# ohsnyt/bzip2-rust

Measured on NVIDIA B200. Metric: compress_MBps_level9_byte_identical, higher is better.
Workload: dtype u8

## Files before the change

bzip2_rust_b200/csrc/bwt.cu:

```cuda
#include "common.cuh"
#include "sweep.cuh"

namespace {

constexpr int FB = 20;
constexpr u64 FMASK = (1ull << FB) - 1;
static_assert(BZ2B200_MAX_BLOCK < (1u << FB) - 1, "packed list fields are 20 bits");

constexpr int RT_IPT = 8;
constexpr int RT = BZ_THREADS * RT_IPT;
__device__ __forceinline__ u32 padi(u32 i) { return i + (i >> 5); }
constexpr int RT_PAD = RT + RT / 32 + 1;

#ifndef BZ_LW
#define BZ_LW 3072
#endif
constexpr int LW = BZ_LW;
constexpr int LIPT = LW / BZ_THREADS;
#ifndef BZ_LCAP
#define BZ_LCAP 1024
#endif
constexpr int LCAP = BZ_LCAP;
constexpr int LTILE = LW - LCAP;
#ifndef BZ_SCAP
#define BZ_SCAP 128
#endif
constexpr int SCAP = BZ_SCAP;
static_assert(LW % BZ_THREADS == 0 && LW <= 4096 && LCAP <= RT && LCAP * 2 <= LW && LCAP <= (1 << 11) && SCAP < LCAP && LW / (SCAP + 1) < 256, "local refinement geometry");
constexpr int LWP = LW + LW / 32 + 1;
__device__ __forceinline__ u32 padh(u32 i) { return i + 2u * (i >> 6); }
constexpr int LWH = LW + 2 * (LW / 64) + 2;

__device__ __forceinline__ u64 rot_key8(const u8 *T, u32 n, u32 s) {
    if (s + 8 <= n) {
        const u64 *w = (const u64 *)(T + (s & ~7u));
        u64 w0 = __ldg(w);
        u32 sh = (s & 7u) * 8u;
        if (sh == 0) return w0;
        u64 w1 = __ldg(w + 1);
        return (w0 >> sh) | (w1 << (64 - sh));
    }
    u64 k = 0;
    u32 p = s;
    for (int q = 0; q < 8; q++) { k |= (u64)T[p] << (8 * q); p++; if (p >= n) p = 0; }
    return k;
}

struct Tri { int a, b; u32 c; };
__device__ __forceinline__ u64 tri_pack(u32 flag, Tri v) {
    return ((u64)flag << 62) | ((u64)(u32)(v.a + 1) << 40) | ((u64)(u32)(v.b + 1) << 20) | (u64)v.c;
}
__device__ __forceinline__ Tri tri_unpack(u64 w) {
    Tri v;
    v.a = (int)((w >> 40) & FMASK) - 1; v.b = (int)((w >> 20) & FMASK) - 1; v.c = (u32)(w & FMASK);
    return v;
}
__device__ __forceinline__ u64 ld_vol64(const u64 *p) {
    u64 v;
    asm volatile("ld.volatile.global.u64 %0, [%1];" : "=l"(v) : "l"(p));
    return v;
}
__device__ __forceinline__ void st_vol64(u64 *p, u64 v) { asm volatile("st.volatile.global.u64 [%0], %1;" ::"l"(p), "l"(v) : "memory"); }

template <bool BSUM = false>
__device__ __forceinline__ Tri tile_lookback(u64 *st, u32 t, Tri agg) {
    const int lane = threadIdx.x & 31;
    const int bid = BSUM ? 0 : -1;
    Tri ex; ex.a = -1; ex.b = bid; ex.c = 0;
    if (t == 0) { if (lane == 0) st_vol64(st, tri_pack(2, agg)); return ex; }
    if (lane == 0) st_vol64(st + t, tri_pack(1, agg));
    for (int hi = (int)t - 1;;) {
        int tt = hi - lane;
        u64 w = tt >= 0 ? ld_vol64(st + tt) : ((2ull << 62) | ((u64)(u32)(bid + 1) << 20));
        u32 f = (u32)(w >> 62);
        u32 incm = __ballot_sync(0xffffffffu, f == 2);
        u32 nrm = __ballot_sync(0xffffffffu, f == 0);
        u32 need = incm ? ((2u << (__ffs(incm) - 1)) - 1u) : 0xffffffffu;
        if (nrm & need) continue;
        Tri v = tri_unpack(w);
        if (!((need >> lane) & 1u)) { v.a = -1; v.b = bid; v.c = 0; }
#pragma unroll
        for (int o = 16; o; o >>= 1) {
            v.a = max(v.a, __shfl_xor_sync(0xffffffffu, v.a, o));
            int ob = __shfl_xor_sync(0xffffffffu, v.b, o);
            v.b = BSUM ? v.b + ob : max(v.b, ob);
            v.c += __shfl_xor_sync(0xffffffffu, v.c, o);
        }
        ex.a = max(ex.a, v.a); ex.b = BSUM ? ex.b + v.b : max(ex.b, v.b); ex.c += v.c;
        if (incm) break;
        hi -= 32;
    }
    Tri inc; inc.a = max(ex.a, agg.a); inc.b = BSUM ? ex.b + agg.b : max(ex.b, agg.b); inc.c = ex.c + agg.c;
    if (lane == 0) st_vol64(st + t, tri_pack(2, inc));
    return ex;
}

struct RefineArgs {
    const u8 *T; const u32 *len;
    const u32 *cnt;
    u32 *SA; u32 *RANK;
    const u64 *LIN; u64 *LOUT;
    u32 *cnt_out;
    u64 *LOUT2;
    u32 *cnt_out2;
    u64 *tstate;
    u32 *ticket;
    u32 stride, rtiles, tiles_x, nblk, group;
    u32 depth_after;
};

__device__ __forceinline__ bool ticket_tile(const RefineArgs &a, u32 *s_ticket, u32 &b, u32 &t) {
    if (threadIdx.x == 0) *s_ticket = atomicAdd(a.ticket, 1u);
    __syncthreads();
    u32 ticket = *s_ticket;
    u32 per_group = a.group * a.tiles_x;
    u32 g = ticket / per_group, r = ticket - g * per_group;
    t = r / a.group;
    b = g * a.group + (r - t * a.group);
    return b < a.nblk;
}

#ifndef BZ_REFINE_MINB
#define BZ_REFINE_MINB 5
#endif
__global__ void __launch_bounds__(BZ_THREADS, BZ_REFINE_MINB) k_init_ranks(RefineArgs a) {
    __shared__ u64 sk[RT + 2];
    __shared__ __align__(8) u8 fl[RT + 8];
    __shared__ u32 hd[RT_PAD];
    __shared__ u16 ls[RT];
    __shared__ int wsi[8];
    __shared__ u32 wsu[8];
    __shared__ u32 s_ticket;
    __shared__ Tri s_ex;
    __shared__ int s_big[2];
    u32 b, t;
    if (!ticket_tile(a, &s_ticket, b, t)) return;
    const u32 n = a.len[b];
    const u32 base = t * RT;
    if (base >= n) return;
    const int tid = threadIdx.x;
    const size_t ob = (size_t)b * a.stride;
    const u8 *Tb = a.T + ob;
    const u32 *sa = a.SA + ob;
    u32 s[RT_IPT];
#pragma unroll
    for (int r = 0; r < RT_IPT; r++) {
        u32 e = r * BZ_THREADS + tid, j = base + e;
        s[r] = 0;
        if (j < n) { s[r] = __ldg(sa + j); sk[e + 1] = rot_key8(Tb, n, s[r]); }
    }
    if (tid == 0 && base > 0) sk[0] = rot_key8(Tb, n, sa[base - 1]);
    if (tid == 32 && base + RT < n) sk[RT + 1] = rot_key8(Tb, n, sa[base + RT]);
    __syncthreads();
    for (u32 e = tid; e <= RT; e += BZ_THREADS) {
        u32 j = base + e;
        fl[e] = (j == 0 || j >= n || sk[e + 1] != sk[e]) ? 1 : 0;
    }
    __syncthreads();
    const u32 eb = tid * RT_IPT;
    const u64 f8 = *(const u64 *)(fl + eb);
    const u32 f9 = fl[eb + 8];
    u32 fm = 0;
#pragma unroll
    for (int r = 0; r < RT_IPT; r++) fm |= (u32)((f8 >> (8 * r)) & 1) << r;
    int last = -1;
    u32 hmask = 0, umask = 0;
#pragma unroll
    for (int r = 0; r < RT_IPT; r++) {
        u32 j = base + eb + r;
        bool h = (fm >> r) & 1;
        bool hn = (r == RT_IPT - 1) ? (f9 != 0) : ((fm >> (r + 1)) & 1);
        if (j < n) {
            if (h) { last = (int)j; hmask |= 1u << r; }
            if (!(h && hn)) umask |= 1u << r;
        }
    }
    int tl, fe;
    int head = block_excl_max(last, wsi, tl);
    int nxa = block_excl_min_rev(fm ? (int)(eb + __ffs(fm) - 1) : 0x7fffffff, wsi, fe);
    const bool cont = fl[RT] == 0;
    if (tid == 64) {
        int big = 0;
        if (fl[0] == 0) {
            if (fe == 0x7fffffff && cont) big = 1;
            else {
                long long E = (long long)base + (fe == 0x7fffffff ? (int)RT : fe);
                long long q = E - 1 - LCAP;
                if (q >= (long long)base) big = 1;
                else if (q >= 0) big = rot_key8(Tb, n, sa[q]) == sk[1];
            }
        }
        s_big[0] = big;
    }
    if (tid == 96) {
        int big = 0;
        if (cont) {
            if (tl < 0) big = 1;
            else {
                u32 P = (u32)tl + LCAP;
                if (P < base + RT) big = 1;
                else if (P < n) big = rot_key8(Tb, n, sa[P]) == sk[RT];
            }
        }
        s_big[1] = big;
    }
    __syncthreads();
    const int nx_out = f9 ? (int)(eb + 8) : (nxa != 0x7fffffff ? nxa : (cont ? 0x7fffffff : (int)RT));
    u32 bmask = 0, nloc = 0, nbig = 0;
#pragma unroll
    for (int r = 0; r < RT_IPT; r++) {
        if ((umask >> r) & 1) {
            u32 below = fm & ((2u << r) - 1u);
            int hh = below ? (int)(base + eb + 31 - __clz(below)) : head;
            u32 above = fm >> (r + 1);
            int nx = above ? (int)(eb + r + __ffs(above)) : nx_out;
            bool big;
            if (hh < 0) big = s_big[0] != 0;
            else if (nx == 0x7fffffff) big = s_big[1] != 0;
            else big = (int)base + nx - hh > LCAP;
            if (big) { bmask |= 1u << r; nbig++; } else nloc++;
        }
    }
    u32 tot;
    u32 kk = block_excl_sum(nloc | (nbig << 16), wsu, tot);
    const u32 tloc = tot & 0xffffu, tbig = tot >> 16;
    if (tid < 32) {
        Tri agg; agg.a = tl; agg.b = (int)tbig; agg.c = tloc;
        Tri ex = tile_lookback<true>(a.tstate + (size_t)b * a.rtiles, t, agg);
        if (tid == 0) {
            s_ex = ex;
            if (base + RT >= n) {
                bool done = a.depth_after >= n;
                a.cnt_out[b] = done ? 0u : ex.c + tloc;
                a.cnt_out2[b] = done ? 0u : (u32)ex.b + tbig;
            }
        }
    }
    __syncthreads();
    head = max(head, s_ex.a);
    u32 kl = kk & 0xffffu, kb = kk >> 16;
#pragma unroll
    for (int r = 0; r < RT_IPT; r++) {
        u32 e = eb + r;
        if ((hmask >> r) & 1) head = (int)(base + e);
        hd[padi(e)] = (u32)head;
        u16 v = 0xffff;
        if ((umask >> r) & 1) v = ((bmask >> r) & 1) ? (u16)(0x8000u | kb++) : (u16)(kl++);
        ls[e] = v;
    }
    __syncthreads();
    u32 *rank = a.RANK + ob;
    u64 *lout = a.LOUT + ob + s_ex.c;
    u64 *lout2 = a.LOUT2 + ob + (u32)s_ex.b;
#pragma unroll
    for (int r = 0; r < RT_IPT; r++) {
        u32 e = r * BZ_THREADS + tid, j = base + e;
        if (j < n) {
            u32 h = hd[padi(e)];
            rank[s[r]] = h;
            u32 slot = ls[e];
            if (slot != 0xffffu) {
                u64 v = ((u64)h << (2 * FB)) | s[r];
                if (slot & 0x8000u) lout2[slot & 0x7fffu] = v; else lout[slot] = v;
            }
        }
    }
}

template <bool HIST>
__global__ void __launch_bounds__(BZ_THREADS) k_list_key(const u32 *cntp, const u32 *len, const u32 *RANK, u64 *LIST,
                                                         u32 *counts, u32 stride, u32 h) {
    u32 b = blockIdx.y, cnt = cntp[b], n = len[b];
    u32 base = blockIdx.x * BZ_TILE;
    if (base >= cnt) return;
    __shared__ u32 hist[HIST ? 5 : 1][256];
    if (HIST) {
        for (int i = threadIdx.x; i < 5 * 256; i += BZ_THREADS) (&hist[0][0])[i] = 0;
        __syncthreads();
    }
    size_t ob = (size_t)b * stride;
    u64 *list = LIST + ob;
    const u32 *rank = RANK + ob;
    u32 hh = h >= n ? h % n : h;
#pragma unroll 4
    for (int r = 0; r < BZ_IPT; r++) {
        u32 k = base + r * BZ_THREADS + threadIdx.x;
        if (k < cnt) {
            u64 x = list[k];
            u32 p = (u32)(x & FMASK) + hh;
            if (p >= n) p -= n;
            x = (x & ~(FMASK << FB)) | ((u64)__ldg(rank + p) << FB);
            list[k] = x;
            if (HIST) {
#pragma unroll
                for (int q = 0; q < 5; q++) atomicAdd(&hist[q][(u32)(x >> (FB + 8 * q)) & 255u], 1u);
            }
        }
    }
    if (HIST) {
        __syncthreads();
        for (int i = threadIdx.x; i < 5 * 256; i += BZ_THREADS) {
            u32 v = (&hist[0][0])[i];
            if (v) atomicAdd(&counts[(size_t)b * 8 * 256 + i], v);
        }
    }
}

__global__ void __launch_bounds__(BZ_THREADS, BZ_REFINE_MINB > 5 ? 5 : BZ_REFINE_MINB) k_list_refine(RefineArgs a) {
    __shared__ u64 sk[RT + 2];
    __shared__ __align__(8) u8 fl[RT + 8];
    __shared__ u32 kgs[RT_PAD], kss[RT_PAD];
    __shared__ u16 ls[RT];
    __shared__ int wsi[8];
    __shared__ u32 wsu[8];
    __shared__ u32 s_ticket;
    __shared__ Tri s_ex;
    u32 b, t;
    if (!ticket_tile(a, &s_ticket, b, t)) return;
    const u32 cnt = a.cnt[b];
    const u32 base = t * RT;
    const int tid = threadIdx.x;
    if (cnt == 0 && t == 0 && tid == 0) a.cnt_out[b] = 0;
    if (base >= cnt) return;
    const size_t ob = (size_t)b * a.stride;
    const u64 *lin = a.LIN + ob;
    u64 x[RT_IPT];
#pragma unroll
    for (int r = 0; r < RT_IPT; r++) {
        u32 e = r * BZ_THREADS + tid, k = base + e;
        x[r] = 0;
        if (k < cnt) { x[r] = __ldg(lin + k); sk[e + 1] = x[r] >> FB; }
    }
    if (tid == 0 && base > 0) sk[0] = lin[base - 1] >> FB;
    if (tid == 32 && base + RT < cnt) sk[RT + 1] = lin[base + RT] >> FB;
    __syncthreads();
    for (u32 e = tid; e <= RT; e += BZ_THREADS) {
        u32 k = base + e;
        u8 f = 3;
        if (k != 0 && k < cnt) {
            u64 c = sk[e + 1], p = sk[e];
            f = (u8)((c != p ? 1 : 0) | ((c >> FB) != (p >> FB) ? 2 : 0));
        }
        fl[e] = f;
    }
    __syncthreads();
    const u32 eb = tid * RT_IPT;
    u64 f8 = *(const u64 *)(fl + eb);
    u32 f9 = fl[eb + 8];
    int la = -1, lb = -1; u32 unres = 0;
    u32 smask = 0, gmask = 0, umask = 0;
#pragma unroll
    for (int r = 0; r < RT_IPT; r++) {
        u32 k = base + eb + r;
        u32 f = (u32)(f8 >> (8 * r)) & 3u;
        u32 fn = (r == RT_IPT - 1) ? f9 : ((u32)(f8 >> (8 * r + 8)) & 3u);
        if (k < cnt) {
            if (f & 2) { la = (int)k; gmask |= 1u << r; }
            if (f & 1) { lb = (int)k; smask |= 1u << r; }
            if (!((f & 1) && (fn & 1))) { unres++; umask |= 1u << r; }
        }
    }
    int ta, tb; u32 tu;
    int kg = block_excl_max(la, wsi, ta);
    int ks = block_excl_max(lb, wsi, tb);
    u32 ko = block_excl_sum(unres, wsu, tu);
    if (tid < 32) {
        Tri agg; agg.a = ta; agg.b = tb; agg.c = tu;
        Tri ex = tile_lookback(a.tstate + (size_t)b * a.rtiles, t, agg);
        if (tid == 0) {
            s_ex = ex;
            if (base + RT >= cnt) a.cnt_out[b] = (a.depth_after >= a.len[b]) ? 0u : ex.c + tu;
        }
    }
    __syncthreads();
    kg = max(kg, s_ex.a); ks = max(ks, s_ex.b);
    const u32 kbase = s_ex.c;
#pragma unroll
    for (int r = 0; r < RT_IPT; r++) {
        u32 e = eb + r;
        if ((gmask >> r) & 1) kg = (int)(base + e);
        if ((smask >> r) & 1) ks = (int)(base + e);
        kgs[padi(e)] = (u32)kg; kss[padi(e)] = (u32)ks;
        ls[e] = ((umask >> r) & 1) ? (u16)(ko++) : (u16)0xffff;
    }
    __syncthreads();
    u32 *sa = a.SA + ob, *rank = a.RANK + ob;
    u64 *lout = a.LOUT + ob + kbase;
#pragma unroll
    for (int r = 0; r < RT_IPT; r++) {
        u32 e = r * BZ_THREADS + tid, k = base + e;
        if (k < cnt) {
            u32 g = (u32)(x[r] >> (2 * FB));
            u32 s = (u32)(x[r] & FMASK);
            u32 kgv = kgs[padi(e)], ksv = kss[padi(e)];
            u32 nh = g + (ksv - kgv);
            sa[g + (k - kgv)] = s;
            rank[s] = nh;
            u32 slot = ls[e];
            if (slot != 0xffffu) lout[slot] = ((u64)nh << (2 * FB)) | s;
        }
    }
}

constexpr size_t LOC_K_BYTES = (size_t)LW * 4;
constexpr size_t LOC_I_BYTES = ((size_t)LWH * 2 + 15) & ~(size_t)15;
constexpr size_t LOC_G_BYTES = ((size_t)LWP * 4 + 15) & ~(size_t)15;
constexpr size_t LOC_U_BYTES = ((size_t)LWH * 2 + 15) & ~(size_t)15;
constexpr size_t LOC_W_BYTES = (size_t)(LW * 4 > 8 * 256 * 4 ? LW * 4 : 8 * 256 * 4);
constexpr size_t LOC_SMEM = LOC_K_BYTES + 2 * LOC_I_BYTES + LOC_G_BYTES + LOC_U_BYTES + LOC_W_BYTES;
static_assert(LOC_K_BYTES + 2 * LOC_I_BYTES >= (size_t)LW * 8, "staging area");
#ifndef BZ_LOCAL_MINB
#define BZ_LOCAL_MINB 3
#endif
__global__ void __launch_bounds__(BZ_THREADS, BZ_LOCAL_MINB) k_refine_local(RefineArgs a, u32 *err) {
    extern __shared__ __align__(16) u8 loc_smem[];
    u32 *K = (u32 *)loc_smem;
    u16 *IDXA = (u16 *)(loc_smem + LOC_K_BYTES);
    u16 *IDXB = (u16 *)(loc_smem + LOC_K_BYTES + LOC_I_BYTES);
    u32 *GSE = (u32 *)(loc_smem + LOC_K_BYTES + 2 * LOC_I_BYTES);
    u16 *UP = (u16 *)((u8 *)GSE + LOC_G_BYTES);
    u32 *wh = (u32 *)((u8 *)UP + LOC_U_BYTES);
    __shared__ u16 MG_GS[LW / (SCAP + 1) + 4], MG_MB[LW / (SCAP + 1) + 4];
    __shared__ int wsi[8];
    __shared__ u32 wsu[8];
    __shared__ u32 s_ticket, s_prevhead;
    __shared__ Tri s_ex;
    u32 b, t;
    if (!ticket_tile(a, &s_ticket, b, t)) return;
    const u32 cnt = a.cnt[b];
    const u32 base = t * LTILE;
    const int tid = threadIdx.x, lane = tid & 31, w = tid >> 5;
    if (cnt == 0 && t == 0 && tid == 0) a.cnt_out[b] = 0;
    if (base >= cnt) return;
    const size_t ob = (size_t)b * a.stride;
    const u64 *lin = a.LIN + ob + base;
    const u32 wlen = min((u32)LW, cnt - base);
    const u32 nom = min((u32)LTILE, cnt - base);
    const int INF = 0x7fffffff;
#pragma unroll 4
    for (int r = 0; r < LIPT; r++) {
        u32 i = r * BZ_THREADS + tid;
        if (i < wlen) {
            u64 x = __ldg(lin + i);
            K[i] = (((u32)(x >> FB) & (u32)FMASK) << 12) | i;
            GSE[padi(i)] = (u32)(x >> (2 * FB));
        }
        UP[padh(i)] = 0xffffu;
    }
    if (tid == 0) s_prevhead = base > 0 ? (u32)(__ldg(lin - 1) >> (2 * FB)) : 0xffffffffu;
    __syncthreads();
    const u32 eb = tid * LIPT;
    u32 gfm = 0;
    {
        u32 prev = tid == 0 ? s_prevhead : GSE[padi(eb - 1)];
#pragma unroll 4
        for (int r = 0; r < LIPT; r++) {
            u32 i = eb + r;
            if (i < wlen) {
                u32 hc = GSE[padi(i)];
                if (hc != prev) gfm |= 1u << r;
                prev = hc;
            }
        }
    }
    int dummy;
    const int gin = block_excl_max(gfm ? (int)(eb + 31 - __clz(gfm)) : -1, wsi, dummy);
    int nout = block_excl_min_rev(gfm ? (int)(eb + __ffs(gfm) - 1) : INF, wsi, dummy);
    if (nout == INF) nout = (int)wlen;
    u32 mcount = 0, mstarts = 0, medmask = 0;
    {
        int ge = nout;
        u32 gem[LIPT];
#pragma unroll
        for (int r = LIPT - 1; r >= 0; r--) {
            gem[r] = (u32)ge;
            if ((gfm >> r) & 1u) ge = (int)(eb + r);
        }
        int gs = gin;
#pragma unroll
        for (int r = 0; r < LIPT; r++) {
            u32 i = eb + r;
            if ((gfm >> r) & 1u) gs = (int)i;
            if (i < wlen) {
                u32 v = 0xffffffffu;
                if (gs >= 0 && gs < (int)nom) {
                    v = (u32)gs | (gem[r] << 16);
                    u32 size = gem[r] - (u32)gs;
                    if (size > (u32)LCAP) atomicOr(err, 1u);
                    if (size > (u32)SCAP) { medmask |= 1u << r; mcount++; if ((u32)gs == i) mstarts++; }
                }
                GSE[padi(i)] = v;
            }
        }
    }
    u32 mtot;
    const u32 mex = block_excl_sum(mcount | (mstarts << 16), wsu, mtot);
    const u32 M = mtot & 0xffffu, nmg = mtot >> 16;
    if (medmask) {
        u32 midx = mex & 0xffffu;
        u32 mgnext = mex >> 16;
#pragma unroll 1
        for (int r = 0; r < LIPT; r++) {
            if ((medmask >> r) & 1u) {
                u32 i = eb + r;
                if ((gfm >> r) & 1u) { MG_GS[mgnext] = (u16)i; MG_MB[mgnext] = (u16)midx; mgnext++; }
                K[i] = ((mgnext - 1u) << FB) | (K[i] >> 12);
                IDXA[padh(midx)] = (u16)i;
                midx++;
            }
        }
    }
    __syncthreads();
#pragma unroll 1
    for (int r = 0; r < LIPT; r++) {
        u32 i = r * BZ_THREADS + tid;
        if (i < wlen) {
            u32 g = GSE[padi(i)];
            u32 gs = g & 0xffffu, ge = g >> 16;
            if (g != 0xffffffffu && ge - gs <= (u32)SCAP) {
                const u32 mine = K[i];
                u32 off = 0;
#pragma unroll 4
                for (u32 q = gs; q < ge; q++) off += K[q] < mine;
                UP[padh(gs + off)] = (u16)i;
            }
        }
    }
    if (M) {
        u16 *src = IDXA, *dst = IDXB;
        const int gb = nmg > 1 ? 32 - __clz((int)nmg - 1) : 0;
        const int passes = (FB + gb + 7) / 8;
        const u32 C = ((M + BZ_THREADS - 1) / BZ_THREADS) * 32;
        const u32 lt = (1u << lane) - 1u;
        u32 *whw = wh + w * 256;
        const u32 j0 = (u32)w * C + lane;
#pragma unroll 1
        for (int p = 0; p < passes; p++) {
            const int shift = 8 * p;
#pragma unroll
            for (int k = 0; k < 8; k++) wh[k * 256 + tid] = 0;
            __syncthreads();
#pragma unroll 1
            for (u32 o = 0; o < C; o += 32) {
                u32 j = j0 + o;
                bool valid = j < M;
                u32 d = valid ? (K[src[padh(j)]] >> shift) & 255u : 256u + (u32)lane;
                u32 peers = __match_any_sync(0xffffffffu, d);
                if (valid && (peers & lt) == 0) whw[d] += __popc(peers);
                __syncwarp();
            }
            __syncthreads();
            {
                u32 c[8], total = 0;
#pragma unroll
                for (int k = 0; k < 8; k++) { c[k] = wh[k * 256 + tid]; total += c[k]; }
                u32 all;
                u32 run = block_excl_sum(total, wsu, all);
#pragma unroll
                for (int k = 0; k < 8; k++) { wh[k * 256 + tid] = run; run += c[k]; }
            }
            __syncthreads();
#pragma unroll 1
            for (u32 o = 0; o < C; o += 32) {
                u32 j = j0 + o;
                bool valid = j < M;
                u32 idx = valid ? (u32)src[padh(j)] : 0u;
                u32 d = valid ? (K[idx] >> shift) & 255u : 256u + (u32)lane;
                u32 peers = __match_any_sync(0xffffffffu, d);
                u32 before = __popc(peers & lt);
                u32 old = 0;
                if (before == 0 && valid) { old = whw[d]; whw[d] = old + __popc(peers); }
                old = __shfl_sync(0xffffffffu, old, __ffs(peers) - 1);
                if (valid) dst[padh(old + before)] = (u16)idx;
                __syncwarp();
            }
            __syncthreads();
            u16 *sw = src; src = dst; dst = sw;
        }
        for (u32 j = tid; j < M; j += BZ_THREADS) {
            u32 i = src[padh(j)];
            u32 g = K[i] >> FB;
            UP[padh((u32)MG_GS[g] + (j - (u32)MG_MB[g]))] = (u16)i;
        }
    }
    __syncthreads();
    u32 tu;
    {
        u32 sfm = 0;
        u32 occ = 0;
        u32 pk = 0xffffffffu;
        if (eb > 0) {
            u32 e = UP[padh(eb - 1)];
            if (e != 0xffffu) { u32 g = GSE[padi(e)]; pk = (g >> 16) - (g & 0xffffu) > (u32)SCAP ? K[e] & (u32)FMASK : K[e] >> 12; }
        }
#pragma unroll 2
        for (int r = 0; r <= LIPT; r++) {
            u32 p = eb + r;
            u32 e = p < (u32)LW ? (u32)UP[padh(p)] : 0xffffu;
            if (e == 0xffffu) { sfm |= 1u << r; pk = 0xffffffffu; continue; }
            u32 g = GSE[padi(e)];
            u32 k2 = (g >> 16) - (g & 0xffffu) > (u32)SCAP ? K[e] & (u32)FMASK : K[e] >> 12;
            if (p == (g & 0xffffu) || k2 != pk) sfm |= 1u << r;
            pk = k2;
            occ |= 1u << r;
        }
        occ &= (1u << LIPT) - 1u;
        const u32 own = sfm & ((1u << LIPT) - 1u);
        const u32 tm = occ & ~(own & (sfm >> 1));
        const int pin = block_excl_max(own ? (int)(eb + 31 - __clz(own)) : -1, wsi, dummy);
        u32 run = block_excl_sum((u32)__popc(tm), wsu, tu);
        int ps = pin;
#pragma unroll 4
        for (int r = 0; r < LIPT; r++) {
            u32 p = eb + r;
            if ((own >> r) & 1u) ps = (int)p;
            wh[p] = run | ((p - (u32)ps) << 12) | (((tm >> r) & 1u) << 31);
            run += (tm >> r) & 1u;
        }
    }
    __syncthreads();
    if (tid < 32) {
        Tri agg; agg.a = -1; agg.b = -1; agg.c = tu;
        Tri ex = tile_lookback(a.tstate + (size_t)b * a.rtiles, t, agg);
        if (tid == 0) {
            s_ex = ex;
            if (base + LTILE >= cnt) a.cnt_out[b] = (a.depth_after >= a.len[b]) ? 0u : ex.c + tu;
        }
    }
    u64 *stg = (u64 *)loc_smem;
    u32 *sa = a.SA + ob, *rank = a.RANK + ob;
#pragma unroll 2
    for (int r = 0; r < LIPT; r++) {
        u32 p = r * BZ_THREADS + tid;
        u32 e = UP[padh(p)];
        if (e != 0xffffu) {
            u32 gs = GSE[padi(e)] & 0xffffu;
            u32 v = wh[p];
            u64 x = __ldg(lin + e);
            u32 head = (u32)(x >> (2 * FB)), s = (u32)(x & FMASK);
            u32 off = p - gs;
            u32 nh = head + off - ((v >> 12) & 0x7ffffu);
            sa[head + off] = s;
            rank[s] = nh;
            if (v >> 31) stg[v & 0xfffu] = ((u64)nh << (2 * FB)) | s;
        }
    }
    __syncthreads();
    u64 *lout = a.LOUT + ob + s_ex.c;
    for (u32 q = tid; q < tu; q += BZ_THREADS) lout[q] = stg[q];
}

__global__ void __launch_bounds__(128) k_ref_path(const u8 *T, const u32 *len, u32 stride, u32 *sais_blocks) {
    const u32 b = blockIdx.x;
    const u32 n = len[b];
    if (n <= 5000) return;
    const u8 *x = T + (size_t)b * stride;
    __shared__ u32 s_cnt;
    if (threadIdx.x == 0) s_cnt = 0;
    __syncthreads();
    const int lo = threadIdx.x * 40;
    u32 lms = 0;
    if (lo < 4999) {
        const int top = min(lo + 40, 4999);
        bool cur_s = false;
        if (top < 4999) {
            u32 c = x[top];
            int j = top + 1;
            while (j <= 4999 && x[j] == c) j++;
            cur_s = j <= 4999 && x[j] > c;
        }
        u32 prev = x[top];
        for (int k = top - 1; k >= lo; k--) {
            u32 el = x[k];
            if (el < prev) cur_s = true;
            else if (el > prev) { if (cur_s) { lms++; cur_s = false; } }
            prev = el;
        }
    }
    lms = __reduce_add_sync(0xffffffffu, lms);
    if ((threadIdx.x & 31) == 0 && lms) atomicAdd(&s_cnt, lms);
    __syncthreads();
    if (threadIdx.x == 0 && s_cnt + 1u <= 1499u) atomicAdd(sais_blocks, 1u);
}

__global__ void __launch_bounds__(256) k_used_from_hist(const u32 *counts, u32 cstride, u32 *usedbits) {
    u32 b = blockIdx.x;
    bool used = counts[(size_t)b * cstride + threadIdx.x] != 0;
    u32 m = __ballot_sync(0xffffffffu, used);
    if ((threadIdx.x & 31) == 0) usedbits[b * 8 + (threadIdx.x >> 5)] = m;
}

__global__ void __launch_bounds__(BZ_THREADS) k_bwt_out(const u8 *T, const u32 *len, const u32 *SA, const u32 *RANK,
                                                        u8 *bwt, u32 *keyout, u32 stride) {
    u32 b = blockIdx.y, n = len[b];
    size_t ob = (size_t)b * stride;
    u32 base = blockIdx.x * BZ_TILE;
    if (blockIdx.x == 0 && threadIdx.x == 0) keyout[b] = n ? RANK[ob] : 0;
#pragma unroll 4
    for (int r = 0; r < BZ_IPT; r++) {
        u32 j = base + r * BZ_THREADS + threadIdx.x;
        if (j < n) {
            u32 s = SA[ob + j];
            bwt[ob + j] = T[ob + (s == 0 ? n - 1 : s - 1)];
        }
    }
}

}

#define LAUNCH_OK()                                                  \
    do {                                                             \
        ctx->prof_end();                                             \
        cudaError_t e_ = cudaGetLastError();                         \
        if (e_ != cudaSuccess) { ctx->fail("kernel launch", e_, __FILE__, __LINE__); return BZ2B200_E_CUDA; } \
    } while (0)

int bz_bwt_batch(bz2b200_ctx *ctx, const Batch &B, u8 *d_bwt, u32 *d_key, u32 *d_usedbits) {
    if (B.nblk == 0) return BZ2B200_OK;
    if (B.max_n > BZ2B200_MAX_BLOCK || ((uintptr_t)B.T & 7u) || (B.stride & 7u)) { ctx->err = "bwt: bad batch geometry"; return BZ2B200_E_ARG; }
    cudaStream_t st = ctx->stream;
    const u64 ne_act = B.total_n;
    const size_t ne = (size_t)B.nblk * B.stride;
    const u32 min_tile = BZ_THREADS * 8;
    const u32 tiles_min = B.stride / min_tile;
    const u32 DSTRIDE = 8 * 256;
    const u32 NTICKET = 512;
    BZ_CHECK(ctx->d_SA.ensure(ne * 4));
    BZ_CHECK(ctx->d_SA2.ensure(ne * 4));
    BZ_CHECK(ctx->d_RANK.ensure(ne * 4));
    BZ_CHECK(ctx->d_KEYA.ensure(ne * 8));
    BZ_CHECK(ctx->d_KEYB.ensure(ne * 8));
    BZ_CHECK(ctx->d_thist.ensure((size_t)B.nblk * tiles_min * 256 * 4));
    BZ_CHECK(ctx->d_tagg.ensure((size_t)B.nblk * tiles_min * 8));
    BZ_CHECK(ctx->d_VALA.ensure(ne * 8));
    BZ_CHECK(ctx->d_VALB.ensure(ne * 8));
    BZ_CHECK(ctx->d_cnt.ensure((size_t)B.nblk * 4 * 4 + 16));
    BZ_CHECK(ctx->d_R.ensure(((size_t)B.nblk * DSTRIDE + NTICKET) * 4));
    BZ_CHECK(ctx->h_small.ensure((size_t)B.nblk * 8 + 64));
    u32 *d_sais = ctx->d_cnt.as<u32>() + (size_t)B.nblk * 4;
    BZ_CHECK(cudaMemsetAsync(d_sais, 0, 8, ctx->stream));
    if (!ctx->loc_attr_done) {
        BZ_CHECK(cudaFuncSetAttribute(k_refine_local, cudaFuncAttributeMaxDynamicSharedMemorySize, (int)LOC_SMEM));
        ctx->loc_attr_done = true;
    }
    u32 *SAa = ctx->d_SA.as<u32>(), *SAb = ctx->d_SA2.as<u32>(), *RANK = ctx->d_RANK.as<u32>();
    u64 *L0 = ctx->d_KEYA.as<u64>(), *L1 = ctx->d_KEYB.as<u64>();
    u64 *G0 = ctx->d_VALA.as<u64>(), *G1 = ctx->d_VALB.as<u64>();
    u32 *tstate = ctx->d_thist.as<u32>();
    u64 *rstate = ctx->d_tagg.as<u64>();
    u32 *dcounts = ctx->d_R.as<u32>();
    u32 *tickets = dcounts + (size_t)B.nblk * DSTRIDE;
    const size_t rstate_bytes = (size_t)B.nblk * tiles_min * 8;

    BZ_CHECK(cudaMemsetAsync(dcounts, 0, ((size_t)B.nblk * DSTRIDE + NTICKET) * 4, st));
    BZ_CHECK(cudaMemsetAsync(tstate, 0, (size_t)B.nblk * tiles_min * 256 * 4, st));
    u32 epoch = 0, tk = 0;
    dim3 gfull((B.max_n + BZ_TILE - 1) / BZ_TILE, B.nblk);
    static const u32 group_knob = [] { const char *e = getenv("BZ2B200_REFINE_GROUP"); u32 g = e ? (u32)atoi(e) : 4u; return g < 1 ? 1u : g; }();
    const u32 group = group_knob < (u32)B.nblk ? group_knob : (u32)B.nblk;

    ctx->prof_begin(K_BYTE_HIST, ne_act); sweep::k_byte_hist<<<gfull, BZ_THREADS, 0, st>>>(B.T, B.len, dcounts, B.stride, DSTRIDE); LAUNCH_OK();
    ctx->prof_begin(K_REF_PATH, (u64)B.nblk * 5000); k_ref_path<<<B.nblk, 128, 0, st>>>(B.T, B.len, B.stride, d_sais); LAUNCH_OK();
    if (d_usedbits) { ctx->prof_begin(K_USED, (u64)B.nblk * 1024); k_used_from_hist<<<B.nblk, 256, 0, st>>>(dcounts, DSTRIDE, d_usedbits); LAUNCH_OK(); }
    ctx->prof_begin(K_DIGIT_SCAN, (u64)B.nblk * DSTRIDE * 4); sweep::k_digit_scan<<<B.nblk * 8, 256, 0, st>>>(dcounts); LAUNCH_OK();
    u32 *bufs[2] = {SAa, SAb};
    const u32 *src = nullptr;
    for (int p = 0; p < 8; p++) {
        sweep::Args a{};
        a.T = B.T; a.len = B.len; a.cnt = B.len; a.in = src; a.out = bufs[p & 1];
        a.stride = B.stride; a.off = 7 - p; a.nblk = (u32)B.nblk;
        epoch++;
        a.dbase = dcounts; a.dbase_stride = DSTRIDE; a.tstate = tstate; a.ticket = tickets + tk++; a.epoch = epoch;
        if ((p & 1) == 0) { ctx->prof_begin(K_SWEEP_GATHER, ne_act * 9); sweep::launch<sweep::M_GATHER>(a, B.max_n, st); }
        else { ctx->prof_begin(K_SWEEP_CARRY, ne_act * 8); sweep::launch<sweep::M_CARRY>(a, B.max_n, st); }
        LAUNCH_OK();
        src = bufs[p & 1];
    }
    u32 *SA = bufs[1];

    u32 *cntL_cur = ctx->d_cnt.as<u32>(), *cntL_nxt = cntL_cur + B.nblk;
    u32 *cntB_cur = cntL_nxt + B.nblk, *cntB_nxt = cntB_cur + B.nblk;
    RefineArgs ra{};
    ra.T = B.T; ra.len = B.len; ra.SA = SA; ra.RANK = RANK; ra.stride = B.stride; ra.rtiles = tiles_min;
    ra.nblk = (u32)B.nblk; ra.group = group; ra.tstate = rstate;
    {
        BZ_CHECK(cudaMemsetAsync(rstate, 0, rstate_bytes, st));
        ra.cnt = B.len; ra.LIN = nullptr; ra.LOUT = L0; ra.cnt_out = cntL_cur; ra.LOUT2 = G0; ra.cnt_out2 = cntB_cur;
        ra.ticket = tickets + tk++;
        ra.tiles_x = (B.max_n + RT - 1) / RT; ra.depth_after = 8;
        u32 grid = ((ra.nblk + group - 1) / group) * group * ra.tiles_x;
        ctx->prof_begin(K_INIT_RANKS, ne_act * 16); k_init_ranks<<<grid, BZ_THREADS, 0, st>>>(ra); LAUNCH_OK();
    }

    u32 *h_cnt = ctx->h_small.as<u32>();
    const int passes = 5;
    u64 rounds = 0, listsum = 0, bigsum = 0;
    for (u32 h = 8;; h *= 2) {
        BZ_CHECK(cudaMemcpyAsync(h_cnt + 2 * B.nblk, d_sais, 8, cudaMemcpyDeviceToHost, st));
        BZ_CHECK(cudaMemcpyAsync(h_cnt, cntL_cur, (size_t)B.nblk * 4, cudaMemcpyDeviceToHost, st));
        BZ_CHECK(cudaMemcpyAsync(h_cnt + B.nblk, cntB_cur, (size_t)B.nblk * 4, cudaMemcpyDeviceToHost, st));
        BZ_CHECK(cudaStreamSynchronize(st));
        u32 maxl = 0, maxb = 0;
        u64 lsum = 0, bsum = 0;
        for (int b = 0; b < B.nblk; b++) {
            if (h_cnt[b] > maxl) maxl = h_cnt[b];
            if (h_cnt[B.nblk + b] > maxb) maxb = h_cnt[B.nblk + b];
            lsum += h_cnt[b]; bsum += h_cnt[B.nblk + b];
        }
        listsum += lsum + bsum; bigsum += bsum;
        if (maxl == 0 && maxb == 0) break;
        if (h >= (1u << 30)) { ctx->err = "bwt: doubling did not terminate"; return BZ2B200_E_CUDA; }
        rounds++;
        if (tk + (u32)passes + 3 > NTICKET) { BZ_CHECK(cudaMemsetAsync(tickets, 0, NTICKET * 4, st)); tk = 0; }
        if (maxl) {
            dim3 gl((maxl + BZ_TILE - 1) / BZ_TILE, B.nblk);
            ctx->prof_begin(K_LIST_KEY, lsum * 20); k_list_key<false><<<gl, BZ_THREADS, 0, st>>>(cntL_cur, B.len, RANK, L0, nullptr, B.stride, h); LAUNCH_OK();
            BZ_CHECK(cudaMemsetAsync(rstate, 0, rstate_bytes, st));
            ra.cnt = cntL_cur; ra.LIN = L0; ra.LOUT = L1; ra.cnt_out = cntL_nxt; ra.LOUT2 = nullptr; ra.cnt_out2 = nullptr;
            ra.ticket = tickets + tk++;
            ra.tiles_x = (maxl + LTILE - 1) / LTILE; ra.depth_after = 2 * h;
            u32 grid = ((ra.nblk + group - 1) / group) * group * ra.tiles_x;
            ctx->prof_begin(K_REFINE_LOCAL, lsum * 24); k_refine_local<<<grid, BZ_THREADS, LOC_SMEM, st>>>(ra, d_sais + 1); LAUNCH_OK();
            { u64 *tl = L0; L0 = L1; L1 = tl; }
        } else BZ_CHECK(cudaMemsetAsync(cntL_nxt, 0, (size_t)B.nblk * 4, st));
        if (maxb) {
            dim3 gl((maxb + BZ_TILE - 1) / BZ_TILE, B.nblk);
            BZ_CHECK(cudaMemsetAsync(dcounts, 0, (size_t)B.nblk * DSTRIDE * 4, st));
            ctx->prof_begin(K_LIST_KEY, bsum * 20); k_list_key<true><<<gl, BZ_THREADS, 0, st>>>(cntB_cur, B.len, RANK, G0, dcounts, B.stride, h); LAUNCH_OK();
            ctx->prof_begin(K_DIGIT_SCAN, (u64)B.nblk * DSTRIDE * 4); sweep::k_digit_scan<<<B.nblk * 8, 256, 0, st>>>(dcounts); LAUNCH_OK();
            if (epoch + (u32)passes > 254) {
                BZ_CHECK(cudaMemsetAsync(tstate, 0, (size_t)B.nblk * tiles_min * 256 * 4, st));
                epoch = 0;
            }
            for (int p = 0; p < passes; p++) {
                sweep::Args a{};
                a.T = B.T; a.len = B.len; a.cnt = cntB_cur; a.in = G0; a.out = G1;
                a.stride = B.stride; a.shift = FB + 8 * p; a.nblk = (u32)B.nblk;
                epoch++;
                a.dbase = dcounts + p * 256; a.dbase_stride = DSTRIDE; a.tstate = tstate; a.ticket = tickets + tk++; a.epoch = epoch;
                ctx->prof_begin(K_SWEEP_LIST, bsum * 16); sweep::launch<sweep::M_LIST>(a, maxb, st); LAUNCH_OK();
                u64 *tl = G0; G0 = G1; G1 = tl;
            }
            BZ_CHECK(cudaMemsetAsync(rstate, 0, rstate_bytes, st));
            ra.cnt = cntB_cur; ra.LIN = G0; ra.LOUT = G1; ra.cnt_out = cntB_nxt; ra.LOUT2 = nullptr; ra.cnt_out2 = nullptr;
            ra.ticket = tickets + tk++;
            ra.tiles_x = (maxb + RT - 1) / RT; ra.depth_after = 2 * h;
            u32 grid = ((ra.nblk + group - 1) / group) * group * ra.tiles_x;
            ctx->prof_begin(K_LIST_REFINE, bsum * 24); k_list_refine<<<grid, BZ_THREADS, 0, st>>>(ra); LAUNCH_OK();
            { u64 *tl = G0; G0 = G1; G1 = tl; }
        } else BZ_CHECK(cudaMemsetAsync(cntB_nxt, 0, (size_t)B.nblk * 4, st));
        { u32 *tc = cntL_cur; cntL_cur = cntL_nxt; cntL_nxt = tc; }
        { u32 *tc = cntB_cur; cntB_cur = cntB_nxt; cntB_nxt = tc; }
    }
    if (h_cnt[2 * B.nblk + 1]) { ctx->err = "bwt: a local group exceeded its capacity"; return BZ2B200_E_CUDA; }
    ctx->prof_begin(K_BWT_OUT, ne_act * 6); k_bwt_out<<<gfull, BZ_THREADS, 0, st>>>(B.T, B.len, SA, RANK, d_bwt, d_key, B.stride); LAUNCH_OK();
    ctx->bwt_stats[0] = (u64)B.nblk; ctx->bwt_stats[1] = ne_act; ctx->bwt_stats[2] = rounds; ctx->bwt_stats[3] = listsum;
    ctx->bwt_stats[4] = h_cnt[2 * B.nblk];
    ctx->bwt_stats[5] += h_cnt[2 * B.nblk];
    ctx->bwt_stats[6] += (u64)B.nblk;
    ctx->bwt_stats[7] = bigsum;
    return BZ2B200_OK;
}
```

bzip2_rust_b200/csrc/common.cuh:

```cuda
#pragma once
#include <cuda_runtime.h>
#include <stdint.h>
#include <stddef.h>
#include <mutex>
#include <string>
#include <vector>
#include <new>
#include "../../include/bz2b200.h"

typedef uint8_t u8;
typedef uint16_t u16;
typedef uint32_t u32;
typedef uint64_t u64;

#define BZ_CHECK(call)                                                                     \
    do {                                                                                   \
        cudaError_t e_ = (call);                                                           \
        if (e_ != cudaSuccess) {                                                           \
            ctx->fail(#call, e_, __FILE__, __LINE__);                                      \
            return BZ2B200_E_CUDA;                                                         \
        }                                                                                  \
    } while (0)

#define BZ_API_TRY try {
#define BZ_API_CATCH } catch (const std::bad_alloc &) { return BZ2B200_E_NOMEM; } catch (...) { return BZ2B200_E_CUDA; }

struct DevBuf {
    void *p = nullptr;
    size_t cap = 0;
    cudaError_t ensure(size_t bytes) {
        if (bytes <= cap) return cudaSuccess;
        if (p) cudaFree(p);
        p = nullptr; cap = 0;
        size_t want = bytes + bytes / 8 + 4096;
        cudaError_t e = cudaMalloc(&p, want);
        if (e == cudaSuccess) cap = want;
        return e;
    }
    void release() { if (p) cudaFree(p); p = nullptr; cap = 0; }
    template <class T> T *as() const { return (T *)p; }
};
struct PinBuf {
    void *p = nullptr;
    size_t cap = 0;
    cudaError_t ensure(size_t bytes) {
        if (bytes <= cap) return cudaSuccess;
        if (p) cudaFreeHost(p);
        p = nullptr; cap = 0;
        size_t want = bytes + bytes / 8 + 4096;
        cudaError_t e = cudaMallocHost(&p, want);
        if (e == cudaSuccess) cap = want;
        return e;
    }
    void release() { if (p) cudaFreeHost(p); p = nullptr; cap = 0; }
    template <class T> T *as() const { return (T *)p; }
};

constexpr int BZ_THREADS = 256;
constexpr int BZ_IPT = 16;
constexpr int BZ_TILE = BZ_THREADS * BZ_IPT;
constexpr int BZ_GROUP = 50;
constexpr int BZ_MAXSYM = 258;

struct Batch {
    int nblk;
    u32 stride;
    u32 tiles;
    u32 max_n;
    int nbits;
    const u8 *T;
    const u32 *len;
    u64 total_n;
};

enum KernelId { K_RADIX_HIST0, K_RADIX_SCAN, K_RADIX_SCATTER0, K_REF_PATH, K_BYTE_HIST, K_DIGIT_SCAN, K_SWEEP_GATHER, K_SWEEP_CARRY, K_SWEEP_LIST, K_INIT_RANKS, K_LIST_KEY, K_LIST_REFINE, K_REFINE_LOCAL, K_BWT_OUT, K_USED, K_MTF_SUMMARY, K_MTF_SCAN, K_MTF_EMIT, K_HUF_INIT, K_HUF_SELECT, K_HUF_LENGTHS, K_HUF_GBITS, K_HUF_LAYOUT, K_HUF_EMIT, K_RLE_SCAN, K_RLE_CHAIN, K_RLE_EMIT, K_CRC_PIECES, K_CRC_FINAL, K_CONCAT, K_FOOTER, K_DEC_MISC, K_DEC_MAGIC, K_DEC_HEADER, K_DEC_JUMPS, K_DEC_BOUNDS, K_DEC_SYMS, K_DEC_CHUNKS, K_DEC_EXPAND, K_DEC_CHUNK_SCAN, K_IBWT_CHASE, K_IBWT_RANK, K_IBWT_WRITE, K_DEC_RLE1_COUNT, K_DEC_RLE1_WRITE, K_COUNT };
static const char *const kKernelNames[] = { "k_radix_hist0", "k_radix_scan", "k_radix_scatter0", "k_ref_path", "k_byte_hist", "k_digit_scan", "k_sweep_gather", "k_sweep_carry", "k_sweep_list", "k_init_ranks", "k_list_key", "k_list_refine", "k_refine_local", "k_bwt_out", "k_used", "k_mtf_summary", "k_mtf_scan", "k_mtf_emit", "k_huf_init", "k_huf_select", "k_huf_lengths", "k_huf_gbits", "k_huf_layout", "k_huf_emit", "k_rle_scan", "k_rle_chain", "k_rle_emit", "k_crc_pieces", "k_crc_final", "k_concat", "k_footer", "k_dec_misc", "k_dec_find_magic", "k_dec_header", "k_dec_jumps", "k_dec_bounds", "k_dec_syms", "k_dec_chunks", "k_dec_expand", "k_dec_chunk_scan", "k_ibwt_chase", "k_ibwt_rank", "k_ibwt_write", "k_dec_rle1_count", "k_dec_rle1_write" };

struct KStat { double ms = 0; u64 launches = 0; u64 bytes = 0; };
struct PendingEv { int id; u64 bytes; cudaEvent_t a, b; };

struct Arrival {
    std::vector<cudaEvent_t> *ev;
    size_t chunk;
    size_t win_off;
    size_t waited;
};

struct ShardPlan {
    bool scanned = false;
    const u8 *d_win = nullptr; size_t win_lo = 0, win_len = 0, n_total = 0; int level = 0;
    bool planned = false;
    bool eof = false; u32 off_from = 0, stop_rel = 0, s0 = 0, nb = 0;
};

struct bz2b200_ctx {
    int device = 0;
    ShardPlan shard;
    cudaStream_t stream = nullptr;
    cudaStream_t s_up = nullptr, s_down = nullptr;
    std::vector<cudaEvent_t> up_ev;
    Arrival *arrival = nullptr;
    std::mutex mu;
    std::string err;
    u64 launches = 0;
    bool timing = false;
    bool dec_attr_done = false;
    bool loc_attr_done = false;
    float stage_ms[8] = {0};
    u64 bwt_stats[8] = {0};
    cudaEvent_t ev[8] = {nullptr};
    cudaEvent_t ev_total[2] = {nullptr, nullptr};
    cudaStream_t s_hi = nullptr;
    cudaEvent_t ev_dec[2] = {nullptr, nullptr};

    DevBuf d_T, d_len, d_crc;
    PinBuf h_stage, h_small, h_out;
    DevBuf d_SA, d_SA2, d_RANK, d_F, d_KEYA, d_KEYB, d_VALA, d_VALB, d_thist, d_tagg, d_cnt, d_bwt, d_key;
    DevBuf d_mtfstate, d_chunkrec, d_R, d_sym, d_m, d_freq, d_used, d_agg2;
    DevBuf d_len6, d_rfreq, d_sel, d_gbits, d_hdr, d_bitoff, d_out, d_outbits, d_hmisc;
    DevBuf d_in, d_runflag, d_misc, d_stream, d_dec1, d_dec2, d_dec3;
    DevBuf d_dwin, d_ddec[2];
    PinBuf h_dstage[2], h_dpiece[2];
    bool dstream_open = false;

    KStat kstat[K_COUNT];
    std::vector<cudaEvent_t> ev_pool;
    std::vector<PendingEv> pending;
    size_t ev_used = 0;
    int cur_id = -1;
    int prof_level = 0;
    cudaEvent_t next_event() {
        if (ev_used == ev_pool.size()) { cudaEvent_t e; cudaEventCreate(&e); ev_pool.push_back(e); }
        return ev_pool[ev_used++];
    }
    void prof_begin(int id, u64 bytes) {
        cur_id = id;
        if (prof_level < 2) return;
        PendingEv p; p.id = id; p.bytes = bytes; p.a = next_event(); p.b = next_event();
        cudaEventRecord(p.a, stream);
        pending.push_back(p);
    }
    void prof_end() {
        launches++;
        if (prof_level < 2 || pending.empty()) return;
        cudaEventRecord(pending.back().b, stream);
    }
    void prof_collect() {
        for (auto &p : pending) {
            float ms = 0;
            if (cudaEventElapsedTime(&ms, p.a, p.b) == cudaSuccess) { kstat[p.id].ms += ms; kstat[p.id].launches++; kstat[p.id].bytes += p.bytes; }
        }
        pending.clear();
        ev_used = 0;
    }

    void fail(const char *what, cudaError_t e, const char *file, int line) {
        err = std::string(what) + ": " + cudaGetErrorString(e) + " at " + file + ":" + std::to_string(line);
    }
    ~bz2b200_ctx();
};

#ifdef __CUDACC__
__device__ __forceinline__ u32 warp_incl_sum(u32 v) {
#pragma unroll
    for (int o = 1; o < 32; o <<= 1) {
        u32 t = __shfl_up_sync(0xffffffffu, v, o);
        if ((threadIdx.x & 31) >= o) v += t;
    }
    return v;
}
__device__ __forceinline__ int warp_incl_max(int v) {
#pragma unroll
    for (int o = 1; o < 32; o <<= 1) {
        int t = __shfl_up_sync(0xffffffffu, v, o);
        if ((threadIdx.x & 31) >= o) v = max(v, t);
    }
    return v;
}
__device__ __forceinline__ u32 block_excl_sum(u32 v, u32 *ws, u32 &total) {
    int lane = threadIdx.x & 31, w = threadIdx.x >> 5;
    u32 inc = warp_incl_sum(v);
    __syncthreads();
    if (lane == 31) ws[w] = inc;
    __syncthreads();
    u32 wsum = (lane < (int)(blockDim.x >> 5)) ? ws[lane] : 0;
    u32 winc = warp_incl_sum(wsum);
    u32 wbase = __shfl_sync(0xffffffffu, winc, w) - __shfl_sync(0xffffffffu, wsum, w);
    total = __shfl_sync(0xffffffffu, winc, (blockDim.x >> 5) - 1);
    return wbase + inc - v;
}
__device__ __forceinline__ int block_excl_max(int v, int *ws, int &total) {
    int lane = threadIdx.x & 31, w = threadIdx.x >> 5;
    int inc = warp_incl_max(v);
    __syncthreads();
    if (lane == 31) ws[w] = inc;
    __syncthreads();
    int wv = (lane < (int)(blockDim.x >> 5)) ? ws[lane] : -1;
    int winc = warp_incl_max(wv);
    int wprev = __shfl_up_sync(0xffffffffu, winc, 1);
    if (lane == 0) wprev = -1;
    int wbase = __shfl_sync(0xffffffffu, wprev, w);
    total = __shfl_sync(0xffffffffu, winc, (blockDim.x >> 5) - 1);
    int prev = __shfl_up_sync(0xffffffffu, inc, 1);
    if (lane == 0) prev = -1;
    return max(wbase, prev);
}
__device__ __forceinline__ int block_excl_min_rev(int v, int *ws, int &total) {
    const int INF = 0x7fffffff;
    int lane = threadIdx.x & 31, w = threadIdx.x >> 5;
    int inc = v;
#pragma unroll
    for (int o = 1; o < 32; o <<= 1) {
        int t = __shfl_down_sync(0xffffffffu, inc, o);
        if (lane + o < 32) inc = min(inc, t);
    }
    __syncthreads();
    if (lane == 0) ws[w] = inc;
    __syncthreads();
    int wv = (lane < (int)(blockDim.x >> 5)) ? ws[lane] : INF;
    int winc = wv;
#pragma unroll
    for (int o = 1; o < 32; o <<= 1) {
        int t = __shfl_down_sync(0xffffffffu, winc, o);
        if (lane + o < 32) winc = min(winc, t);
    }
    int wnext = __shfl_down_sync(0xffffffffu, winc, 1);
    if (lane == 31) wnext = INF;
    int wbase = __shfl_sync(0xffffffffu, wnext, w);
    total = __shfl_sync(0xffffffffu, winc, 0);
    int nxt = __shfl_down_sync(0xffffffffu, inc, 1);
    if (lane == 31) nxt = INF;
    return min(wbase, nxt);
}
#endif

int bz_stage_blocks(bz2b200_ctx *ctx, int nblk, const u8 *const *blk, const u32 *len, Batch &B);
int bz_make_batch_dev(bz2b200_ctx *ctx, int nblk, u32 stride, u32 max_n, const u8 *dT, const u32 *dlen, Batch &B);
int bz_bwt_batch(bz2b200_ctx *ctx, const Batch &B, u8 *d_bwt , u32 *d_key ,
                 u32 *d_usedbits = nullptr);
int bz_mtf_batch(bz2b200_ctx *ctx, const Batch &B, const u8 *d_bwt, u16 *d_sym , u32 *d_m,
                 u32 *d_freq , u8 *d_used , bool used_ready = false);
struct HufOut {
    u8 *d_out;
    u64 *d_bits;
    size_t out_stride;
    u8 *d_len6;
    u8 *d_sel;
    u32 sel_stride;
    u32 *d_ntab;
};
int bz_huf_batch(bz2b200_ctx *ctx, const Batch &B, const u16 *d_sym, const u32 *d_m, const u32 *d_freq,
                 const u8 *d_used, int emit_header, const u32 *d_crc, const u32 *d_key, HufOut &out);

int bz_rle1_window(bz2b200_ctx *ctx, const u8 *d_x, u32 W, int level, bool is_eof, u32 off_from, u32 max_blocks,
                   Batch &B, u32 *nblocks, u32 *consumed, std::vector<u32> *h_spans, bool plan_only,
                   u32 stop_at = 0xFFFFFFFFu, int skip = 0, u32 s0 = 0);
int bz_crc_dev(bz2b200_ctx *ctx, const u8 *d_x, u32 n, u32 *d_crc_out);
int bz_compress_batch(bz2b200_ctx *ctx, const Batch &B, const u32 *d_crc, HufOut &H);
int bz_contexts_on_device(int device);
std::mutex &bz_device_lock(int device);

enum { DEC_BLOCK = 0, DEC_FOOTER = 1, DEC_STREAM = 2 };
struct DecEvent {
    u64 bit;
    u32 val;
    u32 nblock;
    int kind;
};
constexpr long long DEC_ENDED = 1ll << 62;
constexpr int DEC_ABORTED = 1;
struct DecSink {
    virtual long long chain_start() { return -1; }
    virtual void chain_end(long long) {}
    virtual int counted(u64 nbytes, bool last, u8 **d_out, u8 **h_out) = 0;
    virtual int ready(const u8 *, u64) { return BZ2B200_OK; }
    virtual ~DecSink() {}
};
struct DecWindow {
    const u8 *in; size_t in_lo, n;
    const u8 *d_win; size_t lo, len;
    u64 hi_bit;
    long long expect;
    u32 combined;
    u32 max_block;
    const std::vector<u64> *cand;
};
int bz_dec_candidates(bz2b200_ctx *ctx, const u8 *d_win, size_t len, u32 cap, std::vector<u64> &cand);
void bz_add_chance_candidates(std::vector<u64> &cand);
int bz_decode_core(bz2b200_ctx *ctx, const DecWindow &w, DecSink &sink, std::vector<DecEvent> &ev);
int bz_check_block_sizes(std::string &err, int level, const std::vector<DecEvent> &ev);
```

bzip2_rust_b200/csrc/sweep.cuh:

```cuda
#pragma once
#include "common.cuh"
#include <stdlib.h>
#include <type_traits>

namespace sweep {

enum { M_GATHER = 0, M_LIST = 1, M_CARRY = 2 };

struct Args {
    const u8 *T; const u32 *len;
    const u32 *cnt;
    const void *in; void *out;
    const u32 *dbase;
    u32 dbase_stride;
    u32 *tstate;
    u32 *ticket;
    u32 stride;
    u32 rtiles;
    u32 epoch;
    u32 tiles_x;
    u32 nblk;
    u32 group;
    int off;
    int shift;
};

__device__ __forceinline__ u32 ld_vol(const u32 *p) {
    u32 v;
    asm volatile("ld.volatile.global.u32 %0, [%1];" : "=r"(v) : "l"(p));
    return v;
}
__device__ __forceinline__ void st_vol(u32 *p, u32 v) { asm volatile("st.volatile.global.u32 [%0], %1;" ::"l"(p), "r"(v) : "memory"); }

#ifndef BZ_SWEEP_TMA
#define BZ_SWEEP_TMA 0
#endif
__device__ __forceinline__ u32 smem_u32(const void *p) { return (u32)__cvta_generic_to_shared(p); }
__device__ __forceinline__ void mbar_init(u64 *bar, u32 count) {
    asm volatile("mbarrier.init.shared::cta.b64 [%0], %1;" ::"r"(smem_u32(bar)), "r"(count) : "memory");
    asm volatile("fence.mbarrier_init.release.cluster;" ::: "memory");
}
__device__ __forceinline__ void bulk_load(void *dst, const void *src, u32 bytes, u64 *bar) {
    asm volatile("mbarrier.arrive.expect_tx.shared::cta.b64 _, [%0], %1;" ::"r"(smem_u32(bar)), "r"(bytes) : "memory");
    asm volatile("cp.async.bulk.shared::cluster.global.mbarrier::complete_tx::bytes [%0], [%1], %2, [%3];"
                 ::"r"(smem_u32(dst)), "l"(src), "r"(bytes), "r"(smem_u32(bar)) : "memory");
}
__device__ __forceinline__ void mbar_wait(u64 *bar, u32 parity) {
    u32 ok;
    do {
        asm volatile("{\n .reg .pred p;\n mbarrier.try_wait.parity.shared::cta.b64 p, [%1], %2;\n selp.u32 %0, 1, 0, p;\n}"
                     : "=r"(ok) : "r"(smem_u32(bar)), "r"(parity) : "memory");
    } while (!ok);
}

template <int MODE> struct Types { typedef u32 In; typedef u32 Stage; typedef u32 Out; };
template <> struct Types<M_GATHER> { typedef u32 In; typedef u64 Stage; typedef u32 Out; };
template <> struct Types<M_LIST> { typedef u64 In; typedef u64 Stage; typedef u64 Out; };

template <int MODE, int IPT, bool FULL>
__device__ __forceinline__ void tile_body(const Args &a, u32 b, u32 t, u32 base, u32 tile_n, u32 n, u32 *wh, u32 *toff,
                                          u32 *ws, typename Types<MODE>::Stage *sbuf, u64 *bar) {
    typedef typename Types<MODE>::Stage S;
    typedef typename Types<MODE>::Out O;
    const int tid = threadIdx.x, lane = tid & 31, w = tid >> 5;
    const u32 lt = (1u << lane) - 1u;
    const u32 e0 = (u32)w * (32 * IPT) + lane;
    u32 *whw = wh + w * 256;
    typename std::conditional<MODE == M_LIST, u64, u32>::type v[IPT];
    u32 cp[MODE == M_GATHER ? (IPT + 3) / 4 : 1];
    u32 rk[IPT];

    if (MODE == M_GATHER) {
        const u32 *in = a.in ? (const u32 *)a.in + (size_t)b * a.stride + base : nullptr;
        const u8 *Tb = a.T + (size_t)b * a.stride;
        const u32 offm1 = (u32)a.off - 1u;
#pragma unroll
        for (int r = 0; r < IPT; r++) {
            u32 e = e0 + r * 32;
            v[r] = 0;
            if (FULL || e < tile_n) v[r] = in ? __ldg(in + e) : base + e;
        }
#pragma unroll
        for (int q = 0; q < (IPT + 3) / 4; q++) cp[q] = 0;
#pragma unroll
        for (int r = 0; r < IPT; r++) {
            u32 q0 = (u32)v[r] + offm1;
            if (q0 >= n) { q0 -= n; while (q0 >= n) q0 -= n; }
            u64 word = __ldg((const u64 *)(Tb + (q0 & ~7u)));
            u32 sh = (q0 & 7u) * 8u;
            u32 two = (u32)(word >> sh);
            u32 c = two & 255u, d = (two >> 8) & 255u;
            if ((q0 & 7u) == 7u || q0 + 1 >= n) d = __ldg(Tb + (q0 + 1 >= n ? 0u : q0 + 1));
            v[r] = (u32)v[r] | (d << 24);
            cp[r >> 2] |= c << (8 * (r & 3));
        }
    } else if (BZ_SWEEP_TMA && FULL) {
        mbar_wait(bar, 0);
#pragma unroll
        for (int r = 0; r < IPT; r++) v[r] = sbuf[e0 + r * 32];
    } else if (MODE == M_CARRY) {
        const u32 *in = (const u32 *)a.in + (size_t)b * a.stride + base;
#pragma unroll
        for (int r = 0; r < IPT; r++) {
            u32 e = e0 + r * 32;
            v[r] = 0;
            if (FULL || e < tile_n) v[r] = __ldg(in + e);
        }
    } else {
        const u64 *in = (const u64 *)a.in + (size_t)b * a.stride + base;
#pragma unroll
        for (int r = 0; r < IPT; r++) {
            u32 e = e0 + r * 32;
            v[r] = 0;
            if (FULL || e < tile_n) v[r] = __ldg(in + e);
        }
    }
#define SWEEP_DIGIT(x) (MODE == M_LIST ? ((u32)((u64)(x) >> a.shift) & 255u) : ((u32)(x) >> 24))
#pragma unroll
    for (int r = 0; r < IPT; r++) {
        bool valid = FULL || (e0 + r * 32 < tile_n);
        u32 d = SWEEP_DIGIT(v[r]);
        u32 peers = __match_any_sync(0xffffffffu, valid ? d : 256u);
        u32 before = __popc(peers & lt);
        u32 old = 0;
        if (before == 0 && valid) { old = whw[d]; whw[d] = old + __popc(peers); }
        old = __shfl_sync(0xffffffffu, old, __ffs(peers) - 1);
        rk[r] = old + before;
        __syncwarp();
    }
    __syncthreads();
    {
        u32 c[8], total = 0;
#pragma unroll
        for (int k = 0; k < 8; k++) { c[k] = wh[k * 256 + tid]; total += c[k]; }
        const u32 tag = a.epoch << 22;
        u32 *my = a.tstate + ((size_t)b * a.rtiles + t) * 256 + tid;
        if (t == 0) st_vol(my, (2u << 30) | tag | total);
        else st_vol(my, (1u << 30) | tag | total);
        u32 all;
        u32 ex = block_excl_sum(total, ws, all);
        u32 run = ex;
#pragma unroll
        for (int k = 0; k < 8; k++) { wh[k * 256 + tid] = run; run += c[k]; }
        u32 excl = 0;
        if (t != 0) {
            const u32 *p = my - 256;
            for (int tt = (int)t - 1; tt >= 0;) {
                u32 x = ld_vol(p);
                if (((x >> 22) & 255u) != a.epoch || (x >> 30) == 0) continue;
                excl += x & 0x3fffffu;
                if ((x >> 30) == 2u) break;
                tt--; p -= 256;
            }
            st_vol(my, (2u << 30) | tag | (excl + total));
        }
        toff[tid] = a.dbase[(size_t)b * a.dbase_stride + tid] + excl - ex;
    }
    __syncthreads();
#pragma unroll
    for (int r = 0; r < IPT; r++) {
        if (FULL || (e0 + r * 32 < tile_n)) {
            u32 d = SWEEP_DIGIT(v[r]);
            S x = (S)v[r];
            if (MODE == M_GATHER) x = (S)((u64)v[r] | ((u64)((cp[r >> 2] >> (8 * (r & 3))) & 255u) << 32));
            sbuf[whw[d] + rk[r]] = x;
        }
    }
    __syncthreads();
    O *out = (O *)a.out + (size_t)b * a.stride;
#pragma unroll
    for (int r = 0; r < IPT; r++) {
        u32 p = r * BZ_THREADS + tid;
        if (FULL || p < tile_n) {
            S x = sbuf[p];
            u32 d = SWEEP_DIGIT(x);
            O y;
            if (MODE == M_GATHER) y = (O)(((u32)x & 0xffffffu) | ((u32)((u64)x >> 32) << 24));
            else if (MODE == M_CARRY) y = (O)((u32)x & 0xffffffu);
            else y = (O)x;
            out[toff[d] + p] = y;
        }
    }
#undef SWEEP_DIGIT
}

#ifndef BZ_SWEEP_MINB_G
#define BZ_SWEEP_MINB_G 3
#endif
#ifndef BZ_SWEEP_MINB_L
#define BZ_SWEEP_MINB_L 3
#endif
constexpr int min_ctas(int MODE, int IPT) {
    return MODE == M_CARRY ? (IPT <= 8 ? 6 : 4) : (IPT <= 8 ? 4 : (MODE == M_GATHER ? BZ_SWEEP_MINB_G : BZ_SWEEP_MINB_L));
}

template <int MODE, int IPT>
__global__ void __launch_bounds__(BZ_THREADS, min_ctas(MODE, IPT)) k_sweep(Args a) {
    typedef typename Types<MODE>::Stage S;
    constexpr int TILE = BZ_THREADS * IPT;
    __shared__ u32 wh[8 * 256];
    __shared__ u32 toff[256];
    __shared__ u32 ws[8];
    __shared__ __align__(16) S sbuf[TILE];
    __shared__ __align__(8) u64 s_bar;
    __shared__ u32 s_ticket;
    const int tid = threadIdx.x;
    if (tid == 0) {
        s_ticket = atomicAdd(a.ticket, 1u);
        if (BZ_SWEEP_TMA && MODE != M_GATHER) mbar_init(&s_bar, 1);
    }
#pragma unroll
    for (int k = 0; k < 8; k++) wh[k * 256 + tid] = 0;
    __syncthreads();
    u32 ticket = s_ticket;
    u32 per_group = a.group * a.tiles_x;
    u32 g = ticket / per_group, r = ticket - g * per_group;
    u32 t = r / a.group;
    u32 b = g * a.group + (r - t * a.group);
    if (b >= a.nblk) return;
    u32 cnt = a.cnt[b];
    u32 base = t * TILE;
    if (base >= cnt) return;
    u32 n = a.len[b];
    u32 tile_n = min((u32)TILE, cnt - base);
    if (tile_n == (u32)TILE) {
        if (BZ_SWEEP_TMA && MODE != M_GATHER && tid == 0) {
            typedef typename Types<MODE>::In I;
            bulk_load(sbuf, (const I *)a.in + (size_t)b * a.stride + base, (u32)(TILE * sizeof(I)), &s_bar);
        }
        tile_body<MODE, IPT, true>(a, b, t, base, tile_n, n, wh, toff, ws, sbuf, &s_bar);
    } else tile_body<MODE, IPT, false>(a, b, t, base, tile_n, n, wh, toff, ws, sbuf, &s_bar);
}

struct Knobs { int ipt0, ipt1; u32 group, group_stream; };
static inline const Knobs &knobs() {
    static Knobs k = [] {
        Knobs q;
        const char *e;
        q.ipt0 = (e = getenv("BZ2B200_SWEEP_IPT0")) ? atoi(e) : 16;
        q.ipt1 = (e = getenv("BZ2B200_SWEEP_IPT1")) ? atoi(e) : 16;
        q.group = (e = getenv("BZ2B200_SWEEP_GROUP")) ? (u32)atoi(e) : 32u;
        q.group_stream = (e = getenv("BZ2B200_SWEEP_GROUP_STREAM")) ? (u32)atoi(e) : 128u;
        if (q.group_stream < 1) q.group_stream = 1;
        if (q.ipt0 != 8 && q.ipt0 != 16) q.ipt0 = 16;
        if (q.ipt1 != 8 && q.ipt1 != 16) q.ipt1 = 16;
        if (q.group < 1) q.group = 1;
        return q;
    }();
    return k;
}
static inline u32 tile_elems(int mode) { return (u32)(BZ_THREADS * (mode == M_LIST ? knobs().ipt1 : knobs().ipt0)); }

template <int MODE>
static inline void launch(Args a, u32 max_cnt, cudaStream_t st) {
    const Knobs &k = knobs();
    int ipt = MODE == M_LIST ? k.ipt1 : k.ipt0;
    u32 tile = (u32)(BZ_THREADS * ipt);
    a.tiles_x = (max_cnt + tile - 1) / tile;
    a.rtiles = a.stride / tile;
    a.group = MODE == M_GATHER ? k.group : k.group_stream;
    if (a.group > a.nblk) a.group = a.nblk;
    u32 grid = ((a.nblk + a.group - 1) / a.group) * a.group * a.tiles_x;
    if (grid == 0) return;
    if (ipt == 8) k_sweep<MODE, 8><<<grid, BZ_THREADS, 0, st>>>(a);
    else k_sweep<MODE, 16><<<grid, BZ_THREADS, 0, st>>>(a);
}

static __global__ void __launch_bounds__(BZ_THREADS) k_byte_hist(const u8 *T, const u32 *len, u32 *counts, u32 stride,
                                                                  u32 cstride) {
    u32 b = blockIdx.y, n = len[b];
    u32 base = blockIdx.x * BZ_TILE;
    if (base >= n) return;
    __shared__ u32 h[8][256];
    for (int i = threadIdx.x; i < 8 * 256; i += BZ_THREADS) (&h[0][0])[i] = 0;
    __syncthreads();
    const u8 *t = T + (size_t)b * stride;
    int w = threadIdx.x >> 5;
#pragma unroll 4
    for (int r = 0; r < BZ_IPT; r++) {
        u32 i = base + r * BZ_THREADS + threadIdx.x;
        if (i < n) atomicAdd(&h[w][t[i]], 1u);
    }
    __syncthreads();
    u32 s = 0;
#pragma unroll
    for (int k = 0; k < 8; k++) s += h[k][threadIdx.x];
    if (s) atomicAdd(&counts[(size_t)b * cstride + threadIdx.x], s);
}

static __global__ void __launch_bounds__(256) k_digit_scan(u32 *counts) {
    __shared__ u32 ws[8];
    u32 v = counts[(size_t)blockIdx.x * 256 + threadIdx.x], all;
    u32 ex = block_excl_sum(v, ws, all);
    counts[(size_t)blockIdx.x * 256 + threadIdx.x] = ex;
}

}
```

Baseline: 7395.

## Make init-ranks and gather sweep persistent with cp.async prefetch of next tile

Turns k_init_ranks and the gather-mode sweep into persistent kernels that loop over tickets, with the grid capped at the number of resident CTAs. While the current tile is still being processed, each CTA claims its next tile and issues cp.async loads of the text bytes that tile needs into a dynamic shared buffer. The aim is to hide the latency of the random text gathers behind the scan and scatter work of the tile in flight. In exchange it uses more shared memory (occupancy drops, init min blocks go from 5 to 4), adds double-buffered ticket slots and extra syncs, and makes the control flow more complex.

```diff
diff --git a/bzip2_rust_b200/csrc/bwt.cu b/bzip2_rust_b200/csrc/bwt.cu
--- a/bzip2_rust_b200/csrc/bwt.cu
+++ b/bzip2_rust_b200/csrc/bwt.cu
@@ -112,158 +112,198 @@
 __device__ __forceinline__ bool ticket_tile(const RefineArgs &a, u32 *s_ticket, u32 &b, u32 &t) {
     if (threadIdx.x == 0) *s_ticket = atomicAdd(a.ticket, 1u);
     __syncthreads();
-    u32 ticket = *s_ticket;
-    u32 per_group = a.group * a.tiles_x;
-    u32 g = ticket / per_group, r = ticket - g * per_group;
-    t = r / a.group;
-    b = g * a.group + (r - t * a.group);
+    sweep::ticket_to_tile(*s_ticket, a.group, a.tiles_x, b, t);
     return b < a.nblk;
 }
 
-#ifndef BZ_REFINE_MINB
-#define BZ_REFINE_MINB 5
-#endif
-__global__ void __launch_bounds__(BZ_THREADS, BZ_REFINE_MINB) k_init_ranks(RefineArgs a) {
-    __shared__ u64 sk[RT + 2];
-    __shared__ __align__(8) u8 fl[RT + 8];
-    __shared__ u32 hd[RT_PAD];
-    __shared__ u16 ls[RT];
-    __shared__ int wsi[8];
-    __shared__ u32 wsu[8];
-    __shared__ u32 s_ticket;
-    __shared__ Tri s_ex;
-    __shared__ int s_big[2];
-    u32 b, t;
-    if (!ticket_tile(a, &s_ticket, b, t)) return;
-    const u32 n = a.len[b];
-    const u32 base = t * RT;
-    if (base >= n) return;
-    const int tid = threadIdx.x;
+constexpr size_t INIT_KW_BYTES = (size_t)2 * RT * 8;
+constexpr int INIT_MINB = 4;
+static_assert(RT_PAD * 4 + RT * 2 <= (RT + 2) * 8, "hd and ls share sk's space");
+
+__device__ __forceinline__ void init_issue(const RefineArgs &a, u32 b, u32 t, u32 (&s)[RT_IPT], u64 *kw) {
+    const u32 n = a.len[b], base = t * RT;
     const size_t ob = (size_t)b * a.stride;
     const u8 *Tb = a.T + ob;
     const u32 *sa = a.SA + ob;
-    u32 s[RT_IPT];
 #pragma unroll
     for (int r = 0; r < RT_IPT; r++) {
-        u32 e = r * BZ_THREADS + tid, j = base + e;
+        u32 j = base + r * BZ_THREADS + threadIdx.x;
         s[r] = 0;
-        if (j < n) { s[r] = __ldg(sa + j); sk[e + 1] = rot_key8(Tb, n, s[r]); }
-    }
-    if (tid == 0 && base > 0) sk[0] = rot_key8(Tb, n, sa[base - 1]);
-    if (tid == 32 && base + RT < n) sk[RT + 1] = rot_key8(Tb, n, sa[base + RT]);
-    __syncthreads();
-    for (u32 e = tid; e <= RT; e += BZ_THREADS) {
-        u32 j = base + e;
-        fl[e] = (j == 0 || j >= n || sk[e + 1] != sk[e]) ? 1 : 0;
-    }
-    __syncthreads();
-    const u32 eb = tid * RT_IPT;
-    const u64 f8 = *(const u64 *)(fl + eb);
-    const u32 f9 = fl[eb + 8];
-    u32 fm = 0;
-#pragma unroll
-    for (int r = 0; r < RT_IPT; r++) fm |= (u32)((f8 >> (8 * r)) & 1) << r;
-    int last = -1;
-    u32 hmask = 0, umask = 0;
+        if (j < n) s[r] = __ldg(sa + j);
+    }
 #pragma unroll
     for (int r = 0; r < RT_IPT; r++) {
-        u32 j = base + eb + r;
-        bool h = (fm >> r) & 1;
-        bool hn = (r == RT_IPT - 1) ? (f9 != 0) : ((fm >> (r + 1)) & 1);
-        if (j < n) {
-            if (h) { last = (int)j; hmask |= 1u << r; }
-            if (!(h && hn)) umask |= 1u << r;
-        }
-    }
-    int tl, fe;
-    int head = block_excl_max(last, wsi, tl);
-    int nxa = block_excl_min_rev(fm ? (int)(eb + __ffs(fm) - 1) : 0x7fffffff, wsi, fe);
-    const bool cont = fl[RT] == 0;
-    if (tid == 64) {
-        int big = 0;
-        if (fl[0] == 0) {
-            if (fe == 0x7fffffff && cont) big = 1;
-            else {
-                long long E = (long long)base + (fe == 0x7fffffff ? (int)RT : fe);
-                long long q = E - 1 - LCAP;
-                if (q >= (long long)base) big = 1;
-                else if (q >= 0) big = rot_key8(Tb, n, sa[q]) == sk[1];
-            }
-        }
-        s_big[0] = big;
-    }
-    if (tid == 96) {
-        int big = 0;
-        if (cont) {
-            if (tl < 0) big = 1;
-            else {
-                u32 P = (u32)tl + LCAP;
-                if (P < base + RT) big = 1;
-                else if (P < n) big = rot_key8(Tb, n, sa[P]) == sk[RT];
-            }
-        }
-        s_big[1] = big;
-    }
-    __syncthreads();
-    const int nx_out = f9 ? (int)(eb + 8) : (nxa != 0x7fffffff ? nxa : (cont ? 0x7fffffff : (int)RT));
-    u32 bmask = 0, nloc = 0, nbig = 0;
-#pragma unroll
-    for (int r = 0; r < RT_IPT; r++) {
-        if ((umask >> r) & 1) {
-            u32 below = fm & ((2u << r) - 1u);
-            int hh = below ? (int)(base + eb + 31 - __clz(below)) : head;
-            u32 above = fm >> (r + 1);
-            int nx = above ? (int)(eb + r + __ffs(above)) : nx_out;
-            bool big;
-            if (hh < 0) big = s_big[0] != 0;
-            else if (nx == 0x7fffffff) big = s_big[1] != 0;
-            else big = (int)base + nx - hh > LCAP;
-            if (big) { bmask |= 1u << r; nbig++; } else nloc++;
-        }
-    }
-    u32 tot;
-    u32 kk = block_excl_sum(nloc | (nbig << 16), wsu, tot);
-    const u32 tloc = tot & 0xffffu, tbig = tot >> 16;
-    if (tid < 32) {
-        Tri agg; agg.a = tl; agg.b = (int)tbig; agg.c = tloc;
-        Tri ex = tile_lookback<true>(a.tstate + (size_t)b * a.rtiles, t, agg);
-        if (tid == 0) {
-            s_ex = ex;
-            if (base + RT >= n) {
-                bool done = a.depth_after >= n;
-                a.cnt_out[b] = done ? 0u : ex.c + tloc;
-                a.cnt_out2[b] = done ? 0u : (u32)ex.b + tbig;
-            }
-        }
-    }
-    __syncthreads();
-    head = max(head, s_ex.a);
-    u32 kl = kk & 0xffffu, kb = kk >> 16;
-#pragma unroll
-    for (int r = 0; r < RT_IPT; r++) {
-        u32 e = eb + r;
-        if ((hmask >> r) & 1) head = (int)(base + e);
-        hd[padi(e)] = (u32)head;
-        u16 v = 0xffff;
-        if ((umask >> r) & 1) v = ((bmask >> r) & 1) ? (u16)(0x8000u | kb++) : (u16)(kl++);
-        ls[e] = v;
-    }
-    __syncthreads();
-    u32 *rank = a.RANK + ob;
-    u64 *lout = a.LOUT + ob + s_ex.c;
-    u64 *lout2 = a.LOUT2 + ob + (u32)s_ex.b;
-#pragma unroll
-    for (int r = 0; r < RT_IPT; r++) {
-        u32 e = r * BZ_THREADS + tid, j = base + e;
-        if (j < n) {
-            u32 h = hd[padi(e)];
-            rank[s[r]] = h;
-            u32 slot = ls[e];
-            if (slot != 0xffffu) {
-                u64 v = ((u64)h << (2 * FB)) | s[r];
-                if (slot & 0x8000u) lout2[slot & 0x7fffu] = v; else lout[slot] = v;
-            }
-        }
+        u32 e = r * BZ_THREADS + threadIdx.x;
+        if (base + e < n && s[r] + 8 <= n) {
+            const u8 *w = Tb + (s[r] & ~7u);
+            sweep::cp_async8(kw + e, w);
+            if (s[r] & 7u) sweep::cp_async8(kw + RT + e, w + 8);
+        }
+    }
+    sweep::cp_async_commit();
+}
+
+__global__ void __launch_bounds__(BZ_THREADS, INIT_MINB) k_init_ranks(RefineArgs a) {
+    extern __shared__ __align__(16) u64 kw[];
+    __shared__ u64 sk[RT + 2];
+    __shared__ __align__(8) u8 fl[RT + 8];
+    u32 *hd = (u32 *)sk;
+    u16 *ls = (u16 *)(hd + RT_PAD);
+    __shared__ int wsi[8];
+    __shared__ u32 wsu[8];
+    __shared__ u32 s_ticket[2];
+    __shared__ Tri s_ex;
+    __shared__ int s_big[2];
+    const int tid = threadIdx.x;
+    const u32 ntickets = ((a.nblk + a.group - 1) / a.group) * a.group * a.tiles_x;
+    u32 b, t;
+    if (!sweep::take_tile(a.ticket, ntickets, a.group, a.tiles_x, a.nblk, a.len, RT, s_ticket, b, t)) return;
+    u32 s[RT_IPT], ns[RT_IPT];
+    init_issue(a, b, t, s, kw);
+    sweep::cp_async_wait_all();
+    for (u32 it = 1;; it++) {
+        const u32 n = a.len[b];
+        const u32 base = t * RT;
+        const size_t ob = (size_t)b * a.stride;
+        const u8 *Tb = a.T + ob;
+        const u32 *sa = a.SA + ob;
+#pragma unroll
+        for (int r = 0; r < RT_IPT; r++) {
+            u32 e = r * BZ_THREADS + tid, j = base + e;
+            if (j < n) {
+                u64 k;
+                if (s[r] + 8 <= n) {
+                    u32 sh = (s[r] & 7u) * 8u;
+                    k = kw[e];
+                    if (sh) k = (k >> sh) | (kw[RT + e] << (64 - sh));
+                } else k = rot_key8(Tb, n, s[r]);
+                sk[e + 1] = k;
+            }
+        }
+        if (tid == 0 && base > 0) sk[0] = rot_key8(Tb, n, sa[base - 1]);
+        if (tid == 32 && base + RT < n) sk[RT + 1] = rot_key8(Tb, n, sa[base + RT]);
+        __syncthreads();
+        for (u32 e = tid; e <= RT; e += BZ_THREADS) {
+            u32 j = base + e;
+            fl[e] = (j == 0 || j >= n || sk[e + 1] != sk[e]) ? 1 : 0;
+        }
+        __syncthreads();
+        const u32 eb = tid * RT_IPT;
+        const u64 f8 = *(const u64 *)(fl + eb);
+        const u32 f9 = fl[eb + 8];
+        u32 fm = 0;
+#pragma unroll
+        for (int r = 0; r < RT_IPT; r++) fm |= (u32)((f8 >> (8 * r)) & 1) << r;
+        int last = -1;
+        u32 hmask = 0, umask = 0;
+#pragma unroll
+        for (int r = 0; r < RT_IPT; r++) {
+            u32 j = base + eb + r;
+            bool h = (fm >> r) & 1;
+            bool hn = (r == RT_IPT - 1) ? (f9 != 0) : ((fm >> (r + 1)) & 1);
+            if (j < n) {
+                if (h) { last = (int)j; hmask |= 1u << r; }
+                if (!(h && hn)) umask |= 1u << r;
+            }
+        }
+        int tl, fe;
+        int head = block_excl_max(last, wsi, tl);
+        int nxa = block_excl_min_rev(fm ? (int)(eb + __ffs(fm) - 1) : 0x7fffffff, wsi, fe);
+        const bool cont = fl[RT] == 0;
+        if (tid == 64) {
+            int big = 0;
+            if (fl[0] == 0) {
+                if (fe == 0x7fffffff && cont) big = 1;
+                else {
+                    long long E = (long long)base + (fe == 0x7fffffff ? (int)RT : fe);
+                    long long q = E - 1 - LCAP;
+                    if (q >= (long long)base) big = 1;
+                    else if (q >= 0) big = rot_key8(Tb, n, sa[q]) == sk[1];
+                }
+            }
+            s_big[0] = big;
+        }
+        if (tid == 96) {
+            int big = 0;
+            if (cont) {
+                if (tl < 0) big = 1;
+                else {
+                    u32 P = (u32)tl + LCAP;
+                    if (P < base + RT) big = 1;
+                    else if (P < n) big = rot_key8(Tb, n, sa[P]) == sk[RT];
+                }
+            }
+            s_big[1] = big;
+        }
+        __syncthreads();
+        const int nx_out = f9 ? (int)(eb + 8) : (nxa != 0x7fffffff ? nxa : (cont ? 0x7fffffff : (int)RT));
+        u32 bmask = 0, nloc = 0, nbig = 0;
+#pragma unroll
+        for (int r = 0; r < RT_IPT; r++) {
+            if ((umask >> r) & 1) {
+                u32 below = fm & ((2u << r) - 1u);
+                int hh = below ? (int)(base + eb + 31 - __clz(below)) : head;
+                u32 above = fm >> (r + 1);
+                int nx = above ? (int)(eb + r + __ffs(above)) : nx_out;
+                bool big;
+                if (hh < 0) big = s_big[0] != 0;
+                else if (nx == 0x7fffffff) big = s_big[1] != 0;
+                else big = (int)base + nx - hh > LCAP;
+                if (big) { bmask |= 1u << r; nbig++; } else nloc++;
+            }
+        }
+        u32 tot;
+        u32 kk = block_excl_sum(nloc | (nbig << 16), wsu, tot);
+        const u32 tloc = tot & 0xffffu, tbig = tot >> 16;
+        if (tid < 32) {
+            Tri agg; agg.a = tl; agg.b = (int)tbig; agg.c = tloc;
+            Tri ex = tile_lookback<true>(a.tstate + (size_t)b * a.rtiles, t, agg);
+            if (tid == 0) {
+                s_ex = ex;
+                if (base + RT >= n) {
+                    bool done = a.depth_after >= n;
+                    a.cnt_out[b] = done ? 0u : ex.c + tloc;
+                    a.cnt_out2[b] = done ? 0u : (u32)ex.b + tbig;
+                }
+            }
+        }
+        u32 nb, nt;
+        const bool more = sweep::take_tile(a.ticket, ntickets, a.group, a.tiles_x, a.nblk, a.len, RT, s_ticket + (it & 1u), nb, nt);
+        if (more) init_issue(a, nb, nt, ns, kw);
+        head = max(head, s_ex.a);
+        u32 kl = kk & 0xffffu, kb = kk >> 16;
+#pragma unroll
+        for (int r = 0; r < RT_IPT; r++) {
+            u32 e = eb + r;
+            if ((hmask >> r) & 1) head = (int)(base + e);
+            hd[padi(e)] = (u32)head;
+            u16 v = 0xffff;
+            if ((umask >> r) & 1) v = ((bmask >> r) & 1) ? (u16)(0x8000u | kb++) : (u16)(kl++);
+            ls[e] = v;
+        }
+        __syncthreads();
+        u32 *rank = a.RANK + ob;
+        u64 *lout = a.LOUT + ob + s_ex.c;
+        u64 *lout2 = a.LOUT2 + ob + (u32)s_ex.b;
+#pragma unroll
+        for (int r = 0; r < RT_IPT; r++) {
+            u32 e = r * BZ_THREADS + tid, j = base + e;
+            if (j < n) {
+                u32 h = hd[padi(e)];
+                rank[s[r]] = h;
+                u32 slot = ls[e];
+                if (slot != 0xffffu) {
+                    u64 v = ((u64)h << (2 * FB)) | s[r];
+                    if (slot & 0x8000u) lout2[slot & 0x7fffu] = v; else lout[slot] = v;
+                }
+            }
+        }
+        if (!more) return;
+        sweep::cp_async_wait_all();
+#pragma unroll
+        for (int r = 0; r < RT_IPT; r++) s[r] = ns[r];
+        b = nb; t = nt;
+        __syncthreads();
     }
 }
 
@@ -306,6 +346,9 @@
     }
 }
 
+#ifndef BZ_REFINE_MINB
+#define BZ_REFINE_MINB 5
+#endif
 __global__ void __launch_bounds__(BZ_THREADS, BZ_REFINE_MINB > 5 ? 5 : BZ_REFINE_MINB) k_list_refine(RefineArgs a) {
     __shared__ u64 sk[RT + 2];
     __shared__ __align__(8) u8 fl[RT + 8];
@@ -743,6 +786,8 @@
         BZ_CHECK(cudaFuncSetAttribute(k_refine_local, cudaFuncAttributeMaxDynamicSharedMemorySize, (int)LOC_SMEM));
         ctx->loc_attr_done = true;
     }
+    if (!ctx->gather_ctas) BZ_CHECK(sweep::gather_setup(ctx->gather_ctas));
+    if (!ctx->init_ctas) BZ_CHECK(sweep::resident_ctas(k_init_ranks, INIT_KW_BYTES, ctx->init_ctas));
     u32 *SAa = ctx->d_SA.as<u32>(), *SAb = ctx->d_SA2.as<u32>(), *RANK = ctx->d_RANK.as<u32>();
     u64 *L0 = ctx->d_KEYA.as<u64>(), *L1 = ctx->d_KEYB.as<u64>();
     u64 *G0 = ctx->d_VALA.as<u64>(), *G1 = ctx->d_VALB.as<u64>();
@@ -771,8 +816,8 @@
         a.stride = B.stride; a.off = 7 - p; a.nblk = (u32)B.nblk;
         epoch++;
         a.dbase = dcounts; a.dbase_stride = DSTRIDE; a.tstate = tstate; a.ticket = tickets + tk++; a.epoch = epoch;
-        if ((p & 1) == 0) { ctx->prof_begin(K_SWEEP_GATHER, ne_act * 9); sweep::launch<sweep::M_GATHER>(a, B.max_n, st); }
-        else { ctx->prof_begin(K_SWEEP_CARRY, ne_act * 8); sweep::launch<sweep::M_CARRY>(a, B.max_n, st); }
+        if ((p & 1) == 0) { ctx->prof_begin(K_SWEEP_GATHER, ne_act * 9); sweep::launch<sweep::M_GATHER>(a, B.max_n, ctx->gather_ctas, st); }
+        else { ctx->prof_begin(K_SWEEP_CARRY, ne_act * 8); sweep::launch<sweep::M_CARRY>(a, B.max_n, 0, st); }
         LAUNCH_OK();
         src = bufs[p & 1];
     }
@@ -789,7 +834,8 @@
         ra.ticket = tickets + tk++;
         ra.tiles_x = (B.max_n + RT - 1) / RT; ra.depth_after = 8;
         u32 grid = ((ra.nblk + group - 1) / group) * group * ra.tiles_x;
-        ctx->prof_begin(K_INIT_RANKS, ne_act * 16); k_init_ranks<<<grid, BZ_THREADS, 0, st>>>(ra); LAUNCH_OK();
+        if (grid > ctx->init_ctas) grid = ctx->init_ctas;
+        ctx->prof_begin(K_INIT_RANKS, ne_act * 16); k_init_ranks<<<grid, BZ_THREADS, INIT_KW_BYTES, st>>>(ra); LAUNCH_OK();
     }
 
     u32 *h_cnt = ctx->h_small.as<u32>();
@@ -838,7 +884,7 @@
                 a.stride = B.stride; a.shift = FB + 8 * p; a.nblk = (u32)B.nblk;
                 epoch++;
                 a.dbase = dcounts + p * 256; a.dbase_stride = DSTRIDE; a.tstate = tstate; a.ticket = tickets + tk++; a.epoch = epoch;
-                ctx->prof_begin(K_SWEEP_LIST, bsum * 16); sweep::launch<sweep::M_LIST>(a, maxb, st); LAUNCH_OK();
+                ctx->prof_begin(K_SWEEP_LIST, bsum * 16); sweep::launch<sweep::M_LIST>(a, maxb, 0, st); LAUNCH_OK();
                 u64 *tl = G0; G0 = G1; G1 = tl;
             }
             BZ_CHECK(cudaMemsetAsync(rstate, 0, rstate_bytes, st));
diff --git a/bzip2_rust_b200/csrc/common.cuh b/bzip2_rust_b200/csrc/common.cuh
--- a/bzip2_rust_b200/csrc/common.cuh
+++ b/bzip2_rust_b200/csrc/common.cuh
@@ -106,6 +106,7 @@
     bool timing = false;
     bool dec_attr_done = false;
     bool loc_attr_done = false;
+    u32 gather_ctas = 0, init_ctas = 0;
     float stage_ms[8] = {0};
     u64 bwt_stats[8] = {0};
     cudaEvent_t ev[8] = {nullptr};
diff --git a/bzip2_rust_b200/csrc/sweep.cuh b/bzip2_rust_b200/csrc/sweep.cuh
--- a/bzip2_rust_b200/csrc/sweep.cuh
+++ b/bzip2_rust_b200/csrc/sweep.cuh
@@ -56,66 +56,58 @@
 template <int MODE> struct Types { typedef u32 In; typedef u32 Stage; typedef u32 Out; };
 template <> struct Types<M_GATHER> { typedef u32 In; typedef u64 Stage; typedef u32 Out; };
 template <> struct Types<M_LIST> { typedef u64 In; typedef u64 Stage; typedef u64 Out; };
-
-template <int MODE, int IPT, bool FULL>
-__device__ __forceinline__ void tile_body(const Args &a, u32 b, u32 t, u32 base, u32 tile_n, u32 n, u32 *wh, u32 *toff,
-                                          u32 *ws, typename Types<MODE>::Stage *sbuf, u64 *bar) {
+template <int MODE> using Elem = typename std::conditional<MODE == M_LIST, u64, u32>::type;
+constexpr int ncarry(int MODE, int IPT) { return MODE == M_GATHER ? (IPT + 3) / 4 : 1; }
+
+__device__ __forceinline__ void cp_async8(void *dst, const void *src) {
+    asm volatile("cp.async.ca.shared.global [%0], [%1], 8;" ::"r"(smem_u32(dst)), "l"(src) : "memory");
+}
+__device__ __forceinline__ void cp_async4(void *dst, const void *src) {
+    asm volatile("cp.async.ca.shared.global [%0], [%1], 4;" ::"r"(smem_u32(dst)), "l"(src) : "memory");
+}
+__device__ __forceinline__ void cp_async_commit() { asm volatile("cp.async.commit_group;" ::: "memory"); }
+__device__ __forceinline__ void cp_async_wait_all() { asm volatile("cp.async.wait_group 0;" ::: "memory"); }
+
+__device__ __forceinline__ void ticket_to_tile(u32 ticket, u32 group, u32 tiles_x, u32 &b, u32 &t) {
+    u32 per_group = group * tiles_x;
+    u32 g = ticket / per_group, r = ticket - g * per_group;
+    t = r / group;
+    b = g * group + (r - t * group);
+}
+
+__device__ __forceinline__ bool take_tile(u32 *counter, u32 ntickets, u32 group, u32 tiles_x, u32 nblk, const u32 *cnt,
+                                          u32 tile_elems, u32 *slot, u32 &b, u32 &t) {
+    if (threadIdx.x == 0) {
+        u32 k;
+        for (;;) {
+            k = atomicAdd(counter, 1u);
+            if (k >= ntickets) { k = 0xffffffffu; break; }
+            ticket_to_tile(k, group, tiles_x, b, t);
+            if (b < nblk && t * tile_elems < cnt[b]) break;
+        }
+        *slot = k;
+    }
+    __syncthreads();
+    u32 k = *slot;
+    if (k == 0xffffffffu) return false;
+    ticket_to_tile(k, group, tiles_x, b, t);
+    return true;
+}
+
+template <int MODE, int IPT, bool FULL, typename F>
+__device__ __forceinline__ void rank_scatter(const Args &a, u32 b, u32 t, u32 tile_n, const Elem<MODE> (&v)[IPT],
+                                             const u32 (&cp)[ncarry(MODE, IPT)], u32 *wh, u32 *toff, u32 *ws,
+                                             typename Types<MODE>::Stage *sbuf, F &&after_lookback) {
     typedef typename Types<MODE>::Stage S;
     typedef typename Types<MODE>::Out O;
     const int tid = threadIdx.x, lane = tid & 31, w = tid >> 5;
     const u32 lt = (1u << lane) - 1u;
     const u32 e0 = (u32)w * (32 * IPT) + lane;
     u32 *whw = wh + w * 256;
-    typename std::conditional<MODE == M_LIST, u64, u32>::type v[IPT];
-    u32 cp[MODE == M_GATHER ? (IPT + 3) / 4 : 1];
-    u32 rk[IPT];
-
-    if (MODE == M_GATHER) {
-        const u32 *in = a.in ? (const u32 *)a.in + (size_t)b * a.stride + base : nullptr;
-        const u8 *Tb = a.T + (size_t)b * a.stride;
-        const u32 offm1 = (u32)a.off - 1u;
-#pragma unroll
-        for (int r = 0; r < IPT; r++) {
-            u32 e = e0 + r * 32;
-            v[r] = 0;
-            if (FULL || e < tile_n) v[r] = in ? __ldg(in + e) : base + e;
-        }
-#pragma unroll
-        for (int q = 0; q < (IPT + 3) / 4; q++) cp[q] = 0;
-#pragma unroll
-        for (int r = 0; r < IPT; r++) {
-            u32 q0 = (u32)v[r] + offm1;
-            if (q0 >= n) { q0 -= n; while (q0 >= n) q0 -= n; }
-            u64 word = __ldg((const u64 *)(Tb + (q0 & ~7u)));
-            u32 sh = (q0 & 7u) * 8u;
-            u32 two = (u32)(word >> sh);
-            u32 c = two & 255u, d = (two >> 8) & 255u;
-            if ((q0 & 7u) == 7u || q0 + 1 >= n) d = __ldg(Tb + (q0 + 1 >= n ? 0u : q0 + 1));
-            v[r] = (u32)v[r] | (d << 24);
-            cp[r >> 2] |= c << (8 * (r & 3));
-        }
-    } else if (BZ_SWEEP_TMA && FULL) {
-        mbar_wait(bar, 0);
-#pragma unroll
-        for (int r = 0; r < IPT; r++) v[r] = sbuf[e0 + r * 32];
-    } else if (MODE == M_CARRY) {
-        const u32 *in = (const u32 *)a.in + (size_t)b * a.stride + base;
-#pragma unroll
-        for (int r = 0; r < IPT; r++) {
-            u32 e = e0 + r * 32;
-            v[r] = 0;
-            if (FULL || e < tile_n) v[r] = __ldg(in + e);
-        }
-    } else {
-        const u64 *in = (const u64 *)a.in + (size_t)b * a.stride + base;
-#pragma unroll
-        for (int r = 0; r < IPT; r++) {
-            u32 e = e0 + r * 32;
-            v[r] = 0;
-            if (FULL || e < tile_n) v[r] = __ldg(in + e);
-        }
-    }
+    u32 rk[(IPT + 1) / 2];
 #define SWEEP_DIGIT(x) (MODE == M_LIST ? ((u32)((u64)(x) >> a.shift) & 255u) : ((u32)(x) >> 24))
+#pragma unroll
+    for (int r = 0; r < (IPT + 1) / 2; r++) rk[r] = 0;
 #pragma unroll
     for (int r = 0; r < IPT; r++) {
         bool valid = FULL || (e0 + r * 32 < tile_n);
@@ -125,7 +117,7 @@
         u32 old = 0;
         if (before == 0 && valid) { old = whw[d]; whw[d] = old + __popc(peers); }
         old = __shfl_sync(0xffffffffu, old, __ffs(peers) - 1);
-        rk[r] = old + before;
+        rk[r >> 1] |= (old + before) << (16 * (r & 1));
         __syncwarp();
     }
     __syncthreads();
@@ -156,14 +148,14 @@
         }
         toff[tid] = a.dbase[(size_t)b * a.dbase_stride + tid] + excl - ex;
     }
-    __syncthreads();
+    after_lookback();
 #pragma unroll
     for (int r = 0; r < IPT; r++) {
         if (FULL || (e0 + r * 32 < tile_n)) {
             u32 d = SWEEP_DIGIT(v[r]);
             S x = (S)v[r];
             if (MODE == M_GATHER) x = (S)((u64)v[r] | ((u64)((cp[r >> 2] >> (8 * (r & 3))) & 255u) << 32));
-            sbuf[whw[d] + rk[r]] = x;
+            sbuf[whw[d] + ((rk[r >> 1] >> (16 * (r & 1))) & 0xffffu)] = x;
         }
     }
     __syncthreads();
@@ -184,15 +176,142 @@
 #undef SWEEP_DIGIT
 }
 
-#ifndef BZ_SWEEP_MINB_G
-#define BZ_SWEEP_MINB_G 3
-#endif
+template <int MODE, int IPT, bool FULL>
+__device__ __forceinline__ void tile_body(const Args &a, u32 b, u32 t, u32 base, u32 tile_n, u32 *wh, u32 *toff,
+                                          u32 *ws, typename Types<MODE>::Stage *sbuf, u64 *bar) {
+    const int tid = threadIdx.x, lane = tid & 31, w = tid >> 5;
+    const u32 e0 = (u32)w * (32 * IPT) + lane;
+    Elem<MODE> v[IPT];
+    const u32 cp[1] = {0};
+    if (BZ_SWEEP_TMA && FULL) {
+        mbar_wait(bar, 0);
+#pragma unroll
+        for (int r = 0; r < IPT; r++) v[r] = sbuf[e0 + r * 32];
+    } else {
+        const Elem<MODE> *in = (const Elem<MODE> *)a.in + (size_t)b * a.stride + base;
+#pragma unroll
+        for (int r = 0; r < IPT; r++) {
+            u32 e = e0 + r * 32;
+            v[r] = 0;
+            if (FULL || e < tile_n) v[r] = __ldg(in + e);
+        }
+    }
+    rank_scatter<MODE, IPT, FULL>(a, b, t, tile_n, v, cp, wh, toff, ws, sbuf, [] { __syncthreads(); });
+}
+
+__device__ __forceinline__ u32 gather_q0(u32 idx, u32 offm1, u32 n) {
+    u32 q0 = idx + offm1;
+    if (q0 >= n) { q0 -= n; while (q0 >= n) q0 -= n; }
+    return q0;
+}
+
+template <int IPT>
+__device__ __forceinline__ void gather_index(const Args &a, u32 b, u32 base, u32 tile_n, u32 (&idx)[IPT]) {
+    const int tid = threadIdx.x, lane = tid & 31, w = tid >> 5;
+    const u32 e0 = (u32)w * (32 * IPT) + lane;
+    const u32 *in = a.in ? (const u32 *)a.in + (size_t)b * a.stride + base : nullptr;
+#pragma unroll
+    for (int r = 0; r < IPT; r++) {
+        u32 e = e0 + r * 32;
+        idx[r] = 0;
+        if (e < tile_n) idx[r] = in ? __ldg(in + e) : base + e;
+    }
+}
+
+template <int IPT>
+__device__ __forceinline__ void gather_issue(const Args &a, u32 b, u32 base, u32 tile_n, u32 n, u64 *wb) {
+    const int tid = threadIdx.x, lane = tid & 31, w = tid >> 5;
+    const u32 e0 = (u32)w * (32 * IPT) + lane;
+    const u8 *Tb = a.T + (size_t)b * a.stride;
+    const u32 offm1 = (u32)a.off - 1u;
+    u32 idx[IPT];
+    gather_index<IPT>(a, b, base, tile_n, idx);
+#pragma unroll
+    for (int r = 0; r < IPT; r++) {
+        u32 e = e0 + r * 32;
+        if (e < tile_n) {
+            u32 q0 = gather_q0(idx[r], offm1, n);
+            if ((q0 & 7u) != 7u) cp_async8(wb + e, Tb + (q0 & ~7u));
+            else {
+                cp_async4(wb + e, Tb + (q0 - 3u));
+                if (q0 + 1 < n) cp_async4((u32 *)(wb + e) + 1, Tb + (q0 + 1));
+            }
+        }
+    }
+    cp_async_commit();
+}
+
+template <int IPT>
+__device__ __forceinline__ void gather_take(const Args &a, u32 b, u32 base, u32 tile_n, u32 n, const u64 *wb,
+                                            u32 (&v)[IPT], u32 (&cp)[(IPT + 3) / 4]) {
+    const int tid = threadIdx.x, lane = tid & 31, w = tid >> 5;
+    const u32 e0 = (u32)w * (32 * IPT) + lane;
+    const u8 *Tb = a.T + (size_t)b * a.stride;
+    const u32 offm1 = (u32)a.off - 1u;
+    u32 idx[IPT];
+    gather_index<IPT>(a, b, base, tile_n, idx);
+    cp_async_wait_all();
+#pragma unroll
+    for (int q = 0; q < (IPT + 3) / 4; q++) cp[q] = 0;
+#pragma unroll
+    for (int r = 0; r < IPT; r++) {
+        u32 e = e0 + r * 32;
+        v[r] = 0;
+        if (e < tile_n) {
+            u32 q0 = gather_q0(idx[r], offm1, n);
+            u32 sh = (q0 & 7u) == 7u ? 24u : (q0 & 7u) * 8u;
+            u32 two = (u32)(wb[e] >> sh);
+            u32 c = two & 255u, d = (two >> 8) & 255u;
+            if (q0 + 1 >= n) d = __ldg(Tb);
+            v[r] = idx[r] | (d << 24);
+            cp[r >> 2] |= c << (8 * (r & 3));
+        }
+    }
+}
+
+template <int IPT>
+__device__ __forceinline__ void gather_tiles(const Args &a, u32 *wh, u32 *toff, u32 *ws, u64 *sbuf, u64 *wb, u32 *slots) {
+    constexpr u32 TILE = BZ_THREADS * IPT;
+    const int tid = threadIdx.x;
+    const u32 ntickets = ((a.nblk + a.group - 1) / a.group) * a.group * a.tiles_x;
+    u32 b, t;
+    if (!take_tile(a.ticket, ntickets, a.group, a.tiles_x, a.nblk, a.cnt, TILE, slots, b, t)) return;
+    u32 n = a.len[b], tile_n = min(TILE, a.cnt[b] - t * TILE);
+    u32 v[IPT], cp[(IPT + 3) / 4];
+    gather_issue<IPT>(a, b, t * TILE, tile_n, n, wb);
+#pragma unroll
+    for (int k = 0; k < 8; k++) wh[k * 256 + tid] = 0;
+    gather_take<IPT>(a, b, t * TILE, tile_n, n, wb, v, cp);
+    __syncthreads();
+    for (u32 it = 1;; it++) {
+        u32 nb = 0, nt = 0, nn = 0, ntile_n = 0;
+        bool more = false;
+        auto next = [&] {
+            more = take_tile(a.ticket, ntickets, a.group, a.tiles_x, a.nblk, a.cnt, TILE, slots + (it & 1u), nb, nt);
+            if (more) {
+                nn = a.len[nb];
+                ntile_n = min(TILE, a.cnt[nb] - nt * TILE);
+                gather_issue<IPT>(a, nb, nt * TILE, ntile_n, nn, wb);
+            }
+        };
+        if (tile_n == TILE) rank_scatter<M_GATHER, IPT, true>(a, b, t, tile_n, v, cp, wh, toff, ws, sbuf, next);
+        else rank_scatter<M_GATHER, IPT, false>(a, b, t, tile_n, v, cp, wh, toff, ws, sbuf, next);
+        if (!more) return;
+#pragma unroll
+        for (int k = 0; k < 8; k++) wh[k * 256 + tid] = 0;
+        gather_take<IPT>(a, nb, nt * TILE, ntile_n, nn, wb, v, cp);
+        b = nb; t = nt; n = nn; tile_n = ntile_n;
+        __syncthreads();
+    }
+}
+
 #ifndef BZ_SWEEP_MINB_L
 #define BZ_SWEEP_MINB_L 3
 #endif
 constexpr int min_ctas(int MODE, int IPT) {
-    return MODE == M_CARRY ? (IPT <= 8 ? 6 : 4) : (IPT <= 8 ? 4 : (MODE == M_GATHER ? BZ_SWEEP_MINB_G : BZ_SWEEP_MINB_L));
-}
+    return MODE == M_CARRY ? (IPT <= 8 ? 6 : 4) : (IPT <= 8 ? 4 : (MODE == M_GATHER ? 3 : BZ_SWEEP_MINB_L));
+}
+constexpr size_t gather_dyn_smem(int IPT) { return (size_t)BZ_THREADS * IPT * 8; }
 
 template <int MODE, int IPT>
 __global__ void __launch_bounds__(BZ_THREADS, min_ctas(MODE, IPT)) k_sweep(Args a) {
@@ -203,33 +322,46 @@
     __shared__ u32 ws[8];
     __shared__ __align__(16) S sbuf[TILE];
     __shared__ __align__(8) u64 s_bar;
-    __shared__ u32 s_ticket;
+    __shared__ u32 s_ticket[2];
     const int tid = threadIdx.x;
-    if (tid == 0) {
-        s_ticket = atomicAdd(a.ticket, 1u);
-        if (BZ_SWEEP_TMA && MODE != M_GATHER) mbar_init(&s_bar, 1);
-    }
-#pragma unroll
-    for (int k = 0; k < 8; k++) wh[k * 256 + tid] = 0;
-    __syncthreads();
-    u32 ticket = s_ticket;
-    u32 per_group = a.group * a.tiles_x;
-    u32 g = ticket / per_group, r = ticket - g * per_group;
-    u32 t = r / a.group;
-    u32 b = g * a.group + (r - t * a.group);
-    if (b >= a.nblk) return;
-    u32 cnt = a.cnt[b];
-    u32 base = t * TILE;
-    if (base >= cnt) return;
-    u32 n = a.len[b];
-    u32 tile_n = min((u32)TILE, cnt - base);
-    if (tile_n == (u32)TILE) {
-        if (BZ_SWEEP_TMA && MODE != M_GATHER && tid == 0) {
-            typedef typename Types<MODE>::In I;
-            bulk_load(sbuf, (const I *)a.in + (size_t)b * a.stride + base, (u32)(TILE * sizeof(I)), &s_bar);
-        }
-        tile_body<MODE, IPT, true>(a, b, t, base, tile_n, n, wh, toff, ws, sbuf, &s_bar);
-    } else tile_body<MODE, IPT, false>(a, b, t, base, tile_n, n, wh, toff, ws, sbuf, &s_bar);
+    if constexpr (MODE == M_GATHER) {
+        extern __shared__ __align__(16) u64 wb[];
+        gather_tiles<IPT>(a, wh, toff, ws, sbuf, wb, s_ticket);
+    } else {
+        if (tid == 0) {
+            s_ticket[0] = atomicAdd(a.ticket, 1u);
+            if (BZ_SWEEP_TMA) mbar_init(&s_bar, 1);
+        }
+#pragma unroll
+        for (int k = 0; k < 8; k++) wh[k * 256 + tid] = 0;
+        __syncthreads();
+        u32 b, t;
+        ticket_to_tile(s_ticket[0], a.group, a.tiles_x, b, t);
+        if (b >= a.nblk) return;
+        u32 cnt = a.cnt[b];
+        u32 base = t * TILE;
+        if (base >= cnt) return;
+        u32 tile_n = min((u32)TILE, cnt - base);
+        if (tile_n == (u32)TILE) {
+            if (BZ_SWEEP_TMA && tid == 0) {
+                typedef typename Types<MODE>::In I;
+                bulk_load(sbuf, (const I *)a.in + (size_t)b * a.stride + base, (u32)(TILE * sizeof(I)), &s_bar);
+            }
+            tile_body<MODE, IPT, true>(a, b, t, base, tile_n, wh, toff, ws, sbuf, &s_bar);
+        } else tile_body<MODE, IPT, false>(a, b, t, base, tile_n, wh, toff, ws, sbuf, &s_bar);
+    }
+}
+
+template <typename K>
+static inline cudaError_t resident_ctas(K kern, size_t dyn, u32 &ctas) {
+    int dev = 0, sms = 0, per_sm = 0;
+    cudaError_t e = cudaGetDevice(&dev);
+    if (e == cudaSuccess) e = cudaDeviceGetAttribute(&sms, cudaDevAttrMultiProcessorCount, dev);
+    if (e == cudaSuccess) e = cudaFuncSetAttribute(kern, cudaFuncAttributeMaxDynamicSharedMemorySize, (int)dyn);
+    if (e == cudaSuccess) e = cudaOccupancyMaxActiveBlocksPerMultiprocessor(&per_sm, kern, BZ_THREADS, dyn);
+    if (e == cudaSuccess && per_sm < 1) e = cudaErrorInvalidConfiguration;
+    ctas = (u32)sms * (u32)per_sm;
+    return e;
 }
 
 struct Knobs { int ipt0, ipt1; u32 group, group_stream; };
@@ -252,7 +384,7 @@
 static inline u32 tile_elems(int mode) { return (u32)(BZ_THREADS * (mode == M_LIST ? knobs().ipt1 : knobs().ipt0)); }
 
 template <int MODE>
-static inline void launch(Args a, u32 max_cnt, cudaStream_t st) {
+static inline void launch(Args a, u32 max_cnt, u32 gather_ctas, cudaStream_t st) {
     const Knobs &k = knobs();
     int ipt = MODE == M_LIST ? k.ipt1 : k.ipt0;
     u32 tile = (u32)(BZ_THREADS * ipt);
@@ -261,9 +393,17 @@
     a.group = MODE == M_GATHER ? k.group : k.group_stream;
     if (a.group > a.nblk) a.group = a.nblk;
     u32 grid = ((a.nblk + a.group - 1) / a.group) * a.group * a.tiles_x;
+    if (MODE == M_GATHER && grid > gather_ctas) grid = gather_ctas;
     if (grid == 0) return;
-    if (ipt == 8) k_sweep<MODE, 8><<<grid, BZ_THREADS, 0, st>>>(a);
-    else k_sweep<MODE, 16><<<grid, BZ_THREADS, 0, st>>>(a);
+    size_t dyn = MODE == M_GATHER ? gather_dyn_smem(ipt) : 0;
+    if (ipt == 8) k_sweep<MODE, 8><<<grid, BZ_THREADS, dyn, st>>>(a);
+    else k_sweep<MODE, 16><<<grid, BZ_THREADS, dyn, st>>>(a);
+}
+
+static inline cudaError_t gather_setup(u32 &ctas) {
+    int ipt = knobs().ipt0;
+    return ipt == 8 ? resident_ctas(k_sweep<M_GATHER, 8>, gather_dyn_smem(8), ctas)
+                    : resident_ctas(k_sweep<M_GATHER, 16>, gather_dyn_smem(16), ctas);
 }
 
 static __global__ void __launch_bounds__(BZ_THREADS) k_byte_hist(const u8 *T, const u32 *len, u32 *counts, u32 stride,
```

Result: slower. 6292 (median of 6 runs) (-14.9%).
